# davidebarbieri/spgpu

Hardware: AMD Instinct MI355X
Metric: HELL fp64 SpMV GFLOP/s + achieved HBM GB/s (% of roofline), 1 GPU (higher is better)
Workload: dtype f64; 1 GPU; HELL fp64 SpMV (spgpuDhellspmv), 10000000 rows x 32 nnz/row uniform, hackSize 32, columns banded, alpha=1 beta=0 (BASELINE configs[1]); rows=10000000, nnz=320000000, hack_size=32, pattern=banded, parallelism=single GPU

## Files before the change

spgpu_amd/capi.py:

```python
import ctypes as C
import os

_HERE = os.path.dirname(os.path.abspath(__file__))
LIB_PATH = os.environ.get("SPGPU_LIB") or os.path.join(_HERE, "lib", "libspgpu.so")


class MissingNativeLibrary(ImportError):
    pass


if not os.path.exists(LIB_PATH):
    raise MissingNativeLibrary(
        f"{LIB_PATH} not found: build it with `make lib` (or __graft_entry__.build()); "
        "spgpu-amd has no Python or CPU fallback for its kernels")

try:
    import torch
except ImportError:
    pass

lib = C.CDLL(LIB_PATH)

SPGPU_SUCCESS, SPGPU_UNSUPPORTED, SPGPU_UNSPECIFIED, SPGPU_OUTOFMEMORY = 0, 1, 2, 3
TYPE_INT, TYPE_FLOAT, TYPE_DOUBLE, TYPE_COMPLEX_FLOAT, TYPE_COMPLEX_DOUBLE = range(5)


class FloatComplex(C.Structure):
    _fields_ = [("x", C.c_float), ("y", C.c_float)]


class DoubleComplex(C.Structure):
    _fields_ = [("x", C.c_double), ("y", C.c_double)]


class HandleStruct(C.Structure):
    _fields_ = [
        ("currentStream", C.c_void_p), ("defaultStream", C.c_void_p),
        ("device", C.c_int), ("warpSize", C.c_int), ("maxThreadsPerBlock", C.c_int),
        ("maxGridSizeX", C.c_int), ("maxGridSizeY", C.c_int), ("maxGridSizeZ", C.c_int),
        ("multiProcessorCount", C.c_int), ("capabilityMajor", C.c_int), ("capabilityMinor", C.c_int),
    ]


Handle = C.POINTER(HandleStruct)
ptr = C.c_void_p
i32 = C.c_int

SCALAR = {"S": C.c_float, "D": C.c_double, "C": FloatComplex, "Z": DoubleComplex}
REAL = {"S": C.c_float, "D": C.c_double, "C": C.c_float, "Z": C.c_double}
TYPE_CODE = {"S": TYPE_FLOAT, "D": TYPE_DOUBLE, "C": TYPE_COMPLEX_FLOAT, "Z": TYPE_COMPLEX_DOUBLE}


def scalar(letter, value):
    if letter in "SD":
        return SCALAR[letter](float(value))
    v = complex(value)
    return SCALAR[letter](v.real, v.imag)


def _bind(name, restype, argtypes):
    fn = getattr(lib, name)
    fn.restype = restype
    fn.argtypes = argtypes
    return fn


DECLARED = {}


def _decl(name, restype, argtypes):
    DECLARED[name] = (restype, argtypes)
    return _bind(name, restype, argtypes)


spgpuCreate = _decl("spgpuCreate", i32, [C.POINTER(Handle), i32])
spgpuDestroy = _decl("spgpuDestroy", None, [Handle])
spgpuStreamCreate = _decl("spgpuStreamCreate", None, [Handle, C.POINTER(C.c_void_p)])
spgpuStreamDestroy = _decl("spgpuStreamDestroy", None, [C.c_void_p])
spgpuSetStream = _decl("spgpuSetStream", None, [Handle, C.c_void_p])
spgpuGetStream = _decl("spgpuGetStream", C.c_void_p, [Handle])
spgpuSizeOf = _decl("spgpuSizeOf", C.c_size_t, [i32])

hellspmv, ellspmv, hdiaspmv = {}, {}, {}
axpby, maxpby, dot, mdot, nrm2, mnrm2 = {}, {}, {}, {}, {}, {}
for _L, _T in SCALAR.items():
    hellspmv[_L] = _decl(f"spgpu{_L}hellspmv", None,
                         [Handle, ptr, ptr, _T, ptr, ptr, i32, ptr, ptr, ptr, i32, i32, ptr, _T, i32])
    ellspmv[_L] = _decl(f"spgpu{_L}ellspmv", None,
                        [Handle, ptr, ptr, _T, ptr, ptr, i32, i32, ptr, ptr, i32, i32, i32, ptr, _T, i32])
    hdiaspmv[_L] = _decl(f"spgpu{_L}hdiaspmv", None,
                         [Handle, ptr, ptr, _T, ptr, ptr, i32, ptr, i32, i32, ptr, _T])
    axpby[_L] = _decl(f"spgpu{_L}axpby", None, [Handle, ptr, i32, _T, ptr, _T, ptr])
    maxpby[_L] = _decl(f"spgpu{_L}maxpby", None, [Handle, ptr, i32, _T, ptr, _T, ptr, i32, i32])
    dot[_L] = _decl(f"spgpu{_L}dot", _T, [Handle, i32, ptr, ptr])
    mdot[_L] = _decl(f"spgpu{_L}mdot", None, [Handle, ptr, i32, ptr, ptr, i32, i32])
    nrm2[_L] = _decl(f"spgpu{_L}nrm2", REAL[_L], [Handle, i32, ptr])
    mnrm2[_L] = _decl(f"spgpu{_L}mnrm2", None, [Handle, ptr, i32, ptr, i32, i32])

scal, vabs, axy, maxy, axypbz, maxypbz, gath, scat, setscal = {}, {}, {}, {}, {}, {}, {}, {}, {}
asum, amax, masum, mamax = {}, {}, {}, {}
for _L, _T in list(SCALAR.items()) + [("I", C.c_int)]:
    gath[_L] = _decl(f"spgpu{_L}gath", None, [Handle, ptr, i32, ptr, i32, ptr])
    scat[_L] = _decl(f"spgpu{_L}scat", None, [Handle, ptr, i32, ptr, ptr, i32, _T])
    setscal[_L] = _decl(f"spgpu{_L}setscal", None, [Handle, i32, i32, i32, _T, ptr])
    if _L == "I":
        continue
    scal[_L] = _decl(f"spgpu{_L}scal", None, [Handle, ptr, i32, _T, ptr])
    vabs[_L] = _decl(f"spgpu{_L}abs", None, [Handle, ptr, i32, _T, ptr])
    axy[_L] = _decl(f"spgpu{_L}axy", None, [Handle, ptr, i32, _T, ptr, ptr])
    maxy[_L] = _decl(f"spgpu{_L}maxy", None, [Handle, ptr, i32, _T, ptr, ptr, i32, i32])
    axypbz[_L] = _decl(f"spgpu{_L}axypbz", None, [Handle, ptr, i32, _T, ptr, _T, ptr, ptr])
    maxypbz[_L] = _decl(f"spgpu{_L}maxypbz", None, [Handle, ptr, i32, _T, ptr, _T, ptr, ptr, i32, i32])
    asum[_L] = _decl(f"spgpu{_L}asum", REAL[_L], [Handle, i32, ptr])
    amax[_L] = _decl(f"spgpu{_L}amax", REAL[_L], [Handle, i32, ptr])
    masum[_L] = _decl(f"spgpu{_L}masum", None, [Handle, ptr, i32, ptr, i32, i32])
    mamax[_L] = _decl(f"spgpu{_L}mamax", None, [Handle, ptr, i32, ptr, i32, i32])

hellspmm, mv_interleave, mv_deinterleave = {}, {}, {}
for _L in "SD":
    _T = SCALAR[_L]
    hellspmm[_L] = _decl(f"spgpu{_L}hellspmm", None,
                         [Handle, ptr, ptr, _T, ptr, ptr, i32, ptr, ptr, ptr, i32, i32, ptr, _T, i32, i32, i32, i32])
    mv_interleave[_L] = _decl(f"spgpu{_L}mvInterleave", None, [Handle, ptr, i32, ptr, i32, i32, i32])
    mv_deinterleave[_L] = _decl(f"spgpu{_L}mvDeinterleave", None, [Handle, ptr, i32, ptr, i32, i32, i32])

hellspmm_mv = {}
for _L in "SD":
    _T = SCALAR[_L]
    hellspmm_mv[_L] = _decl(f"spgpu{_L}hellspmmMv", None,
                            [Handle, ptr, ptr, _T, ptr, ptr, i32, ptr, ptr, ptr, i32, i32, ptr, _T, i32, i32, i32, i32])

computeEllRowLenghts = _decl("computeEllRowLenghts", None, [ptr, C.POINTER(i32), i32, i32, ptr, i32])
computeEllAllocPitch = _decl("computeEllAllocPitch", i32, [i32])
cooToEll = _decl("cooToEll", None, [ptr, ptr, i32, i32, i32, i32, i32, i32, ptr, ptr, ptr, i32, i32])
computeHellAllocSize = _decl("computeHellAllocSize", None, [C.POINTER(i32), i32, i32, ptr])
ellToHell = _decl("ellToHell", None, [ptr, ptr, ptr, i32, ptr, ptr, i32, i32, ptr, i32, i32])
getHdiaHacksCount = _decl("getHdiaHacksCount", i32, [i32, i32])
computeHdiaHackOffsetsFromCoo = _decl("computeHdiaHackOffsetsFromCoo", None,
                                      [C.POINTER(i32), ptr, i32, i32, i32, i32, ptr, ptr, i32])
cooToHdia = _decl("cooToHdia", None, [ptr, ptr, ptr, i32, i32, i32, i32, ptr, ptr, ptr, i32, i32])


diaspmv, ellcsput = {}, {}
for _L, _T in SCALAR.items():
    diaspmv[_L] = _decl(f"spgpu{_L}diaspmv", None, [Handle, ptr, ptr, _T, ptr, ptr, i32, i32, i32, i32, ptr, _T])
    ellcsput[_L] = _decl(f"spgpu{_L}ellcsput", None, [Handle, _T, ptr, ptr, i32, i32, ptr, i32, ptr, ptr, ptr, i32])
computeDiaAllocPitch = _decl("computeDiaAllocPitch", i32, [i32])
computeDiaDiagonalsCount = _decl("computeDiaDiagonalsCount", i32, [i32, i32, i32, ptr, ptr])
coo2dia = _decl("coo2dia", None, [ptr, ptr, i32, i32, i32, i32, i32, ptr, ptr, ptr, i32, i32])
computeHdiaHackOffsets = _decl("computeHdiaHackOffsets", None, [C.POINTER(i32), ptr, i32, ptr, i32, i32, i32, i32])
diaToHdia = _decl("diaToHdia", None, [ptr, ptr, ptr, i32, ptr, ptr, i32, i32, i32, i32])
ellToOell = _decl("ellToOell", None, [ptr, ptr, ptr, ptr, ptr, ptr, ptr, i32, i32, i32, i32])


spgpuCooConvertWorkBytes = _decl("spgpuCooConvertWorkBytes", C.c_size_t, [i32, i32])
spgpuCooRowLengthsDevice = _decl("spgpuCooRowLengthsDevice", i32, [Handle, ptr, C.POINTER(i32), i32, i32, ptr, i32, ptr])
spgpuCooToEllDevice = _decl("spgpuCooToEllDevice", i32, [Handle, ptr, ptr, i32, i32, i32, i32, i32, ptr, ptr, ptr, i32, i32, ptr, ptr])
spgpuHellPlanDevice = _decl("spgpuHellPlanDevice", i32, [Handle, C.POINTER(i32), ptr, i32, i32, ptr, ptr])
spgpuCooToHellDevice = _decl("spgpuCooToHellDevice", i32, [Handle, ptr, ptr, ptr, i32, i32, i32, i32, ptr, ptr, ptr, i32, i32, ptr, ptr])
spgpuCooDiaWorkBytes = _decl("spgpuCooDiaWorkBytes", C.c_size_t, [i32, i32])
spgpuCooDiaPlanDevice = _decl("spgpuCooDiaPlanDevice", i32, [Handle, C.POINTER(i32), i32, i32, i32, ptr, ptr, i32, ptr])
spgpuCooToDiaScratchBytes = _decl("spgpuCooToDiaScratchBytes", C.c_size_t, [i32, i32])
spgpuCooToDiaDevice = _decl("spgpuCooToDiaDevice", i32, [Handle, ptr, ptr, i32, i32, i32, i32, i32, ptr, ptr, ptr, i32, i32, ptr, ptr])
spgpuCooHdiaPlanWorkBytes = _decl("spgpuCooHdiaPlanWorkBytes", C.c_size_t, [i32, i32])
spgpuCooHdiaPlanDevice = _decl("spgpuCooHdiaPlanDevice", i32, [Handle, C.POINTER(i32), ptr, i32, i32, i32, i32, ptr, ptr, i32, ptr])
spgpuCooToHdiaScratchBytes = _decl("spgpuCooToHdiaScratchBytes", C.c_size_t, [i32, i32])
spgpuCooToHdiaDevice = _decl("spgpuCooToHdiaDevice", i32, [Handle, ptr, ptr, ptr, i32, i32, i32, i32, ptr, ptr, ptr, i32, i32, i32, ptr, ptr])


spgpuCsrRowLengthsDevice = _decl("spgpuCsrRowLengthsDevice", i32, [Handle, ptr, C.POINTER(i32), i32, ptr, i32])
spgpuCsrToEllDevice = _decl("spgpuCsrToEllDevice", i32, [Handle, ptr, ptr, i32, i32, i32, i32, ptr, ptr, ptr, i32, i32, ptr])
spgpuCsrToHellDevice = _decl("spgpuCsrToHellDevice", i32, [Handle, ptr, ptr, ptr, i32, i32, i32, ptr, ptr, ptr, i32, i32, ptr])
CSR_FILL_PLAIN, CSR_FILL_TRANSPOSE = 0, 1
spgpuCsrToEllDeviceWith = _bind("spgpuCsrToEllDeviceWith", i32, spgpuCsrToEllDevice.argtypes + [i32, i32])
spgpuCsrToHellDeviceWith = _bind("spgpuCsrToHellDeviceWith", i32, spgpuCsrToHellDevice.argtypes + [i32, i32])
CSR_FILL_CHUNK = _bind("spgpuCsrFillChunk", i32, [])()
CSR_FILL_DEFAULT = _bind("spgpuCsrDefaultFill", i32, [])()


oellOrder = _decl("oellOrder", None, [ptr, ptr, ptr, i32, i32, i32])
oellOrderAligned = _decl("oellOrderAligned", None, [ptr, ptr, ptr, i32, i32, i32])
spgpuOellOrderWorkBytes = _decl("spgpuOellOrderWorkBytes", C.c_size_t, [i32])
spgpuOellOrderDevice = _decl("spgpuOellOrderDevice", i32, [Handle, ptr, ptr, ptr, i32, i32, i32, ptr])
spgpuOellOrderAlignedDevice = _decl("spgpuOellOrderAlignedDevice", i32, [Handle, ptr, ptr, ptr, i32, i32, i32, ptr])
spgpuEllToOellDevice = _decl("spgpuEllToOellDevice", i32, [Handle, ptr, ptr, ptr, ptr, ptr, ptr, ptr, i32, i32, i32, i32, i32, i32, ptr])
spgpuCooPermuteRowsDevice = _decl("spgpuCooPermuteRowsDevice", i32, [Handle, ptr, ptr, i32, ptr, i32, i32, ptr])


class HellBlockD(C.Structure):
    _fields_ = [("cM", C.c_void_p), ("rP", C.c_void_p), ("hackSize", C.c_int), ("hackOffsets", C.c_void_p), ("rS", C.c_void_p),
                ("rows", C.c_int), ("avgNnzPerRow", C.c_int), ("baseIndex", C.c_int), ("slots", C.c_longlong)]


EXCHANGE_ALLGATHER, EXCHANGE_NEEDED = 0, 1
ShardedPlan = C.c_void_p
spgpuCommAvailable = _decl("spgpuCommAvailable", i32, [])
spgpuCommGetUniqueId = _decl("spgpuCommGetUniqueId", i32, [ptr])
spgpuCommInitRank = _decl("spgpuCommInitRank", i32, [C.POINTER(C.c_void_p), i32, ptr, i32])
spgpuCommInitAll = _decl("spgpuCommInitAll", i32, [C.POINTER(C.c_void_p), i32, ptr])
spgpuCommDestroy = _decl("spgpuCommDestroy", None, [ptr])
spgpuDhellspmmShardedCreate = _decl("spgpuDhellspmmShardedCreate", i32,
                                    [C.POINTER(ShardedPlan), Handle, ptr, i32, i32, C.POINTER(C.c_longlong), C.POINTER(HellBlockD),
                                     C.POINTER(HellBlockD), i32, i32])
spgpuDhellspmmShardedStep = _decl("spgpuDhellspmmShardedStep", i32, [ShardedPlan, ptr, ptr, C.c_double, ptr, C.c_double])
spgpuDhellspmmShardedExchange = _decl("spgpuDhellspmmShardedExchange", i32, [ShardedPlan, ptr])
spgpuDhellspmmShardedExchangeWait = _decl("spgpuDhellspmmShardedExchangeWait", i32, [ShardedPlan])
spgpuDhellspmmShardedProducts = _decl("spgpuDhellspmmShardedProducts", i32, [ShardedPlan, ptr, ptr, C.c_double, ptr, C.c_double])
spgpuDhellspmmShardedRowsReceived = _decl("spgpuDhellspmmShardedRowsReceived", C.c_longlong, [ShardedPlan])
spgpuDhellspmmShardedExchanged = _decl("spgpuDhellspmmShardedExchanged", C.c_void_p, [ShardedPlan, C.POINTER(C.c_longlong)])
spgpuDhellspmmShardedDestroy = _decl("spgpuDhellspmmShardedDestroy", None, [ShardedPlan])


def hell_block(part, avg_nnz=0):
    p = lambda t: t.data_ptr()
    slots = int(part["slots"]) if "slots" in part else int(part["cM"].numel())
    return HellBlockD(p(part["cM"]), p(part["rP"]), part["hack_size"], p(part["hack_offsets"]), p(part["rS"]), part["rows"], avg_nnz,
                      part.get("base", 0), slots)


spgpuMmProperties = _decl("spgpuMmProperties", i32, [C.c_char_p, ptr])
spgpuMmReadCoo = _decl("spgpuMmReadCoo", i32, [C.c_char_p, C.c_char, ptr, ptr, ptr])
spgpuMmUnfoldedSizeD = _decl("spgpuMmUnfoldedSizeD", i32, [ptr, ptr, ptr, i32])
spgpuMmUnfoldD = _decl("spgpuMmUnfoldD", None, [ptr, ptr, ptr, ptr, ptr, ptr, i32])


dot_device, axpby_device, axpby_quot_device, div_device, nrm2_device = {}, {}, {}, {}, {}
for _L in "SD":
    dot_device[_L] = _decl(f"spgpu{_L}dotDevice", None, [Handle, ptr, i32, ptr, ptr])
    nrm2_device[_L] = _decl(f"spgpu{_L}nrm2Device", None, [Handle, ptr, i32, ptr])
    axpby_device[_L] = _decl(f"spgpu{_L}axpbyDevice", None, [Handle, ptr, i32, ptr, ptr, ptr, ptr])
    axpby_quot_device[_L] = _decl(f"spgpu{_L}axpbyQuotDevice", None, [Handle, ptr, i32, ptr, ptr, ptr, ptr, ptr, i32, ptr])
    div_device[_L] = _decl(f"spgpu{_L}divDevice", None, [Handle, ptr, ptr, ptr, i32])
hellspmv_dot_device, axpby_pair_dot_device = {}, {}
for _L in "SD":
    _S = SCALAR[_L]
    hellspmv_dot_device[_L] = _decl(f"spgpu{_L}hellspmvDotDevice", None,
                                    [Handle, ptr, ptr, ptr, ptr, _S, ptr, ptr, i32, ptr, ptr, i32, ptr, _S, i32])
    axpby_pair_dot_device[_L] = _decl(f"spgpu{_L}axpbyPairDotDevice", None,
                                      [Handle, ptr, i32, ptr, ptr, ptr, ptr, ptr, ptr, ptr, ptr])


FORM_AUTO, FORM_GATHER, FORM_STRIPS, FORM_XTILE, FORM_SWEEP = range(5)
spgpuSetSpmvForm = _decl("spgpuSetSpmvForm", None, [Handle, i32])
spgpuGetSpmvForm = _decl("spgpuGetSpmvForm", i32, [Handle])
spgpuDeepListOverflows = _decl("spgpuDeepListOverflows", i32, [Handle])
spgpuDeepListFallbacks = _decl("spgpuDeepListFallbacks", i32, [Handle])
spgpuDeepListsRecycled = _decl("spgpuDeepListsRecycled", i32, [Handle])
spgpuSpmvPlanCounts = _decl("spgpuSpmvPlanCounts", None, [Handle, C.POINTER(i32), C.POINTER(i32), C.POINTER(i32)])
spgpuHellSpmvPrepare = _decl("spgpuHellSpmvPrepare", i32, [Handle, i32, ptr, ptr, i32, ptr, ptr, ptr, i32, i32])
spgpuHellSpmvFreeze = _decl("spgpuHellSpmvFreeze", i32, [Handle, i32, ptr, ptr, i32, ptr, ptr, ptr, i32, i32])
spgpuEllSpmvFreeze = _decl("spgpuEllSpmvFreeze", i32, [Handle, i32, ptr, ptr, i32, i32, ptr, ptr, i32, i32, i32])
spgpuHellSpmvAdopt = _decl("spgpuHellSpmvAdopt", i32, [Handle, i32, ptr, ptr, i32, ptr, ptr, i32, i32])
spgpuEllSpmvAdopt = _decl("spgpuEllSpmvAdopt", i32, [Handle, i32, ptr, ptr, i32, i32, ptr, i32, i32, i32])
spgpuHellSpmvOptimize = _decl("spgpuHellSpmvOptimize", i32, [Handle, i32, ptr, ptr, i32, ptr, ptr, ptr, i32, i32])
SPMV_AS_IS, SPMV_FROZEN, SPMV_ADOPTED = 0, 1, 2
spgpuSpmvAdoptedUses = _decl("spgpuSpmvAdoptedUses", i32, [Handle])
spgpuSpmvThaw = _decl("spgpuSpmvThaw", i32, [Handle, ptr])
spgpuSpmvFrozenBytes = _decl("spgpuSpmvFrozenBytes", C.c_longlong, [Handle])
spgpuEllSpmvPrepare = _decl("spgpuEllSpmvPrepare", i32, [Handle, i32, ptr, ptr, i32, i32, ptr, ptr, i32, i32, i32])

SPGPU_IN_USE = 4
spgpuSpmvHold = _decl("spgpuSpmvHold", i32, [Handle, ptr])
spgpuSpmvRelease = _decl("spgpuSpmvRelease", i32, [Handle, ptr])
spgpuSpmvHolds = _decl("spgpuSpmvHolds", i32, [Handle, ptr])


def plan_counts(handle):
    u, b, s = i32(0), i32(0), i32(0)
    spgpuSpmvPlanCounts(handle, C.byref(u), C.byref(b), C.byref(s))
    return u.value, b.value, s.value
spgpuGetLastSpmvForm = _decl("spgpuGetLastSpmvForm", i32, [Handle])
spgpuTuningVariantsBuilt = _decl("spgpuTuningVariantsBuilt", i32, [])
spgpuHellSpmvForm = _decl("spgpuHellSpmvForm", i32, [Handle, i32, ptr, i32, ptr, ptr, i32, i32])
spgpuEllSpmvForm = _decl("spgpuEllSpmvForm", i32, [Handle, i32, ptr, i32, ptr, i32, i32, i32])

spgpuTuningReload = _decl("spgpuTuningReload", None, [])


def create_handle(device=0):
    h = Handle()
    status = spgpuCreate(C.byref(h), device)
    if status != SPGPU_SUCCESS or not h:
        raise RuntimeError(f"spgpuCreate(device={device}) failed with status {status}")
    return h
```

spgpu_amd/csrc/core.c:

```c
#include "spgpu_internal.h"

#include <stdio.h>
#include <stdlib.h>
#include <string.h>

#define DEEP_HEAD_BYTES (SPGPU_DEEP_HEAD_INTS * sizeof(int))
#define DEEP_ENTRY_BYTES ((size_t)SPGPU_DEEP_ENTRIES * sizeof(SpgpuDeepEntry))
#define DEEP_ITEM_ENTRY_BYTES ((size_t)SPGPU_DEEP_ITEMS * sizeof(SpgpuDeepItem))
#define DEEP_PARTIAL_BYTES ((size_t)SPGPU_DEEP_ENTRIES * 32 * 16)
#define DEEP_ITEM_SUM_BYTES ((size_t)SPGPU_DEEP_ITEMS * 32 * 16)

static void deepListFor(SpgpuPrivateHandle* h, hipStream_t stream)
{
    pthread_mutex_lock(&h->tablesLock);
    int known = 0;
    for (int i = 0; i < h->deepStreams; ++i)
        known |= h->deepStream[i] == stream;
    if (!known && h->deepStreams < SPGPU_DEEP_STREAMS) {
        void* p = NULL;
        hipEvent_t idle = NULL;
        if (hipMalloc(&p, DEEP_HEAD_BYTES + DEEP_ENTRY_BYTES + DEEP_ITEM_ENTRY_BYTES + DEEP_PARTIAL_BYTES + DEEP_ITEM_SUM_BYTES) == hipSuccess) {
            if (spgpuTuning()->poisonScratch)
                (void)hipMemset((char*)p + DEEP_HEAD_BYTES + DEEP_ENTRY_BYTES + DEEP_ITEM_ENTRY_BYTES, 0xFF, DEEP_PARTIAL_BYTES + DEEP_ITEM_SUM_BYTES);
            if (hipMemset(p, 0, DEEP_HEAD_BYTES + DEEP_ENTRY_BYTES + DEEP_ITEM_ENTRY_BYTES) == hipSuccess &&
                hipEventCreateWithFlags(&idle, hipEventDisableTiming) == hipSuccess) {
                h->deepScratch[h->deepStreams] = p;
                h->deepStream[h->deepStreams] = stream;
                h->deepIdle[h->deepStreams] = idle;
                h->deepUsed[h->deepStreams] = 0;
                h->deepPinned[h->deepStreams] = 0;
                h->deepClock[h->deepStreams] = ++h->deepTick;
                h->deepStreams += 1;
            } else {
                hipFree(p);
            }
        }
    } else if (!known) {
        int pick = -1;
        for (int i = 0; i < h->deepStreams; ++i) {
            if (h->deepStream[i] == h->pub.defaultStream || h->deepPinned[i])
                continue;
            if (h->deepUsed[i] && !spgpuEventDone(h->deepIdle[i]))
                continue;
            if (pick < 0 || h->deepClock[i] < h->deepClock[pick])
                pick = i;
        }
        if (pick >= 0) {
            h->deepStream[pick] = stream;
            h->deepUsed[pick] = 0;
            h->deepClock[pick] = ++h->deepTick;
            h->deepRecycled += 1;
        }
    }
    pthread_mutex_unlock(&h->tablesLock);
}

spgpuStatus_t spgpuCreate(spgpuHandle_t* pHandle, int device)
{
    if (!pHandle)
        return SPGPU_UNSPECIFIED;
    *pHandle = NULL;

    hipDeviceProp_t prop;
    hipError_t perr = hipGetDeviceProperties(&prop, device);
    if (perr != hipSuccess) {
        fprintf(stderr, "spgpuCreate: hipGetDeviceProperties(%d) failed: %s\n", device, hipGetErrorString(perr));
        return SPGPU_UNSPECIFIED;
    }

    SpgpuPrivateHandle* h = (SpgpuPrivateHandle*)calloc(1, sizeof(SpgpuPrivateHandle));
    if (!h)
        return SPGPU_OUTOFMEMORY;

    int previous = 0;
    hipGetDevice(&previous);
    hipError_t err = hipSetDevice(device);
    if (err == hipSuccess)
        err = hipStreamCreate(&h->pub.defaultStream);
    if (err == hipSuccess)
        err = hipMalloc(&h->reduceScratch, SPGPU_REDUCE_SCRATCH_BYTES);
    if (err == hipSuccess && spgpuTuning()->poisonScratch)
        err = hipMemset(h->reduceScratch, 0xFF, SPGPU_REDUCE_SCRATCH_BYTES);
    if (err == hipSuccess)
        err = hipHostMalloc(&h->reduceHost, SPGPU_REDUCE_SCRATCH_BYTES, hipHostMallocDefault);
    if (err == hipSuccess)
        err = hipHostMalloc((void**)&h->formFeedback, (SPGPU_FEEDBACK_ENTRIES + 2) * SPGPU_FEEDBACK_SAMPLES * sizeof(int),
                            hipHostMallocDefault);
    if (err == hipSuccess)
        memset(h->formFeedback, 0, (SPGPU_FEEDBACK_ENTRIES + 2) * SPGPU_FEEDBACK_SAMPLES * sizeof(int));
    hipSetDevice(previous);

    if (err != hipSuccess) {
        fprintf(stderr, "spgpuCreate: device %d setup failed: %s\n", device, hipGetErrorString(err));
        if (h->reduceScratch) hipFree(h->reduceScratch);
        if (h->reduceHost) hipHostFree(h->reduceHost);
        if (h->pub.defaultStream) hipStreamDestroy(h->pub.defaultStream);
        free(h);
        return err == hipErrorOutOfMemory ? SPGPU_OUTOFMEMORY : SPGPU_UNSPECIFIED;
    }

    h->pub.currentStream = h->pub.defaultStream;
    h->pub.device = device;
    h->pub.warpSize = prop.warpSize;
    h->pub.maxThreadsPerBlock = prop.maxThreadsPerBlock;
    h->pub.maxGridSizeX = prop.maxGridSize[0];
    h->pub.maxGridSizeY = prop.maxGridSize[1];
    h->pub.maxGridSizeZ = prop.maxGridSize[2];
    h->pub.multiProcessorCount = prop.multiProcessorCount;
    h->pub.capabilityMajor = prop.major;
    h->pub.capabilityMinor = prop.minor;
    h->magic = SPGPU_HANDLE_MAGIC;
    pthread_mutex_init(&h->tablesLock, NULL);
    h->spmvForm = SPGPU_SPMV_FORM_AUTO;
    hipSetDevice(device);
    deepListFor(h, h->pub.defaultStream);
    spgpuRecordsCreate(h);
    hipSetDevice(previous);

    *pHandle = &h->pub;
    return SPGPU_SUCCESS;
}

void spgpuDestroy(spgpuHandle_t pHandle)
{
    if (!pHandle)
        return;
    SpgpuPrivateHandle* h = spgpuPrivate(pHandle);
    int previous = 0;
    hipGetDevice(&previous);
    hipSetDevice(h->pub.device);
    hipDeviceSynchronize();
    hipFree(h->reduceScratch);
    for (int i = 0; i < h->deepStreams; ++i) {
        hipFree(h->deepScratch[i]);
        hipEventDestroy(h->deepIdle[i]);
    }
    spgpuRecordsDestroy(h);
    hipHostFree(h->reduceHost);
    hipHostFree(h->formFeedback);
    hipStreamDestroy(h->pub.defaultStream);
    hipSetDevice(previous);
    pthread_mutex_destroy(&h->tablesLock);
    h->magic = 0;
    free(h);
}

void spgpuStreamCreate(spgpuHandle_t pHandle, hipStream_t* stream)
{
    int previous = 0;
    hipGetDevice(&previous);
    hipSetDevice(pHandle->device);
    hipStreamCreate(stream);
    hipSetDevice(previous);
}

void spgpuStreamDestroy(hipStream_t stream)
{
    hipStreamDestroy(stream);
}

void spgpuSetStream(spgpuHandle_t pHandle, hipStream_t stream)
{
    SpgpuPrivateHandle* h = spgpuPrivate(pHandle);
    h->pub.currentStream = stream ? stream : h->pub.defaultStream;
    int known = 0;
    pthread_mutex_lock(&h->tablesLock);
    for (int i = 0; i < h->deepStreams; ++i)
        known |= h->deepStream[i] == h->pub.currentStream;
    pthread_mutex_unlock(&h->tablesLock);
    if (!known) {
        int previous = 0;
        hipGetDevice(&previous);
        hipSetDevice(h->pub.device);
        deepListFor(h, h->pub.currentStream);
        hipSetDevice(previous);
    }
}

hipStream_t spgpuGetStream(spgpuHandle_t pHandle)
{
    return pHandle->currentStream;
}

size_t spgpuSizeOf(spgpuType_t typeCode)
{
    switch (typeCode) {
    case SPGPU_TYPE_INT:            return sizeof(int);
    case SPGPU_TYPE_FLOAT:          return sizeof(float);
    case SPGPU_TYPE_DOUBLE:         return sizeof(double);
    case SPGPU_TYPE_COMPLEX_FLOAT:  return sizeof(hipFloatComplex);
    case SPGPU_TYPE_COMPLEX_DOUBLE: return sizeof(hipDoubleComplex);
    default:                        return 0;
    }
}

spgpuStatus_t spgpuDeepScratch(spgpuHandle_t pHandle, SpgpuDeepList* list)
{
    SpgpuPrivateHandle* h = spgpuPrivate(pHandle);
    char* base = NULL;
    pthread_mutex_lock(&h->tablesLock);
    for (int i = 0; i < h->deepStreams; ++i)
        if (h->deepStream[i] == h->pub.currentStream) {
            base = (char*)h->deepScratch[i];
            list->idle = h->deepIdle[i];
            h->deepUsed[i] = 1;
            h->deepClock[i] = ++h->deepTick;
        }
    if (!base)
        h->deepFallbacks += 1;
    pthread_mutex_unlock(&h->tablesLock);
    if (!base)
        return SPGPU_UNSUPPORTED;
    list->header = (int*)base;
    list->entries = (SpgpuDeepEntry*)(base + DEEP_HEAD_BYTES);
    list->items = (SpgpuDeepItem*)(base + DEEP_HEAD_BYTES + DEEP_ENTRY_BYTES);
    list->partials = base + DEEP_HEAD_BYTES + DEEP_ENTRY_BYTES + DEEP_ITEM_ENTRY_BYTES;
    list->itemSums = base + DEEP_HEAD_BYTES + DEEP_ENTRY_BYTES + DEEP_ITEM_ENTRY_BYTES + DEEP_PARTIAL_BYTES;
    return SPGPU_SUCCESS;
}

void spgpuDeepListPin(spgpuHandle_t pHandle)
{
    SpgpuPrivateHandle* h = spgpuPrivate(pHandle);
    pthread_mutex_lock(&h->tablesLock);
    for (int i = 0; i < h->deepStreams; ++i)
        if (h->deepStream[i] == h->pub.currentStream)
            h->deepPinned[i] = 1;
    pthread_mutex_unlock(&h->tablesLock);
}

int* spgpuAnalyseWords(spgpuHandle_t pHandle)
{
    return spgpuPrivate(pHandle)->formFeedback + SPGPU_FEEDBACK_ENTRIES * SPGPU_FEEDBACK_SAMPLES;
}

int* spgpuDeepOverflowWords(spgpuHandle_t pHandle)
{
    return spgpuPrivate(pHandle)->formFeedback + (SPGPU_FEEDBACK_ENTRIES + 1) * SPGPU_FEEDBACK_SAMPLES;
}

int spgpuDeepListOverflows(spgpuHandle_t pHandle)
{
    return ((volatile int*)spgpuDeepOverflowWords(pHandle))[0];
}

int spgpuDeepListFallbacks(spgpuHandle_t pHandle)
{
    SpgpuPrivateHandle* h = spgpuPrivate(pHandle);
    pthread_mutex_lock(&h->tablesLock);
    const int n = h->deepFallbacks;
    pthread_mutex_unlock(&h->tablesLock);
    return n;
}

int spgpuDeepListsRecycled(spgpuHandle_t pHandle)
{
    SpgpuPrivateHandle* h = spgpuPrivate(pHandle);
    pthread_mutex_lock(&h->tablesLock);
    const int n = h->deepRecycled;
    pthread_mutex_unlock(&h->tablesLock);
    return n;
}

void spgpuSetSpmvForm(spgpuHandle_t pHandle, int form)
{
    if (form < SPGPU_SPMV_FORM_AUTO || form > SPGPU_SPMV_FORM_SWEEP)
        form = SPGPU_SPMV_FORM_AUTO;
    __atomic_store_n(&spgpuPrivate(pHandle)->spmvForm, form, __ATOMIC_RELAXED);
}

int spgpuGetSpmvForm(spgpuHandle_t pHandle)
{
    return __atomic_load_n(&spgpuPrivate(pHandle)->spmvForm, __ATOMIC_RELAXED);
}

int spgpuGetLastSpmvForm(spgpuHandle_t pHandle)
{
    return __atomic_load_n(&spgpuPrivate(pHandle)->lastSpmvForm, __ATOMIC_RELAXED);
}

void spgpuNoteSpmvForm(spgpuHandle_t pHandle, int form)
{
    __atomic_store_n(&spgpuPrivate(pHandle)->lastSpmvForm, form, __ATOMIC_RELAXED);
}

static SpgpuTuning tuning;
static int tuningLoaded;

static int envInt(const char* name, int fallback)
{
    const char* s = getenv(name);
    return s && *s ? atoi(s) : fallback;
}

void spgpuTuningReload(void)
{
    SpgpuTuning t;
    t.xStrips = envInt("SPGPU_X_STRIPS", -1);
    t.autoSweep = envInt("SPGPU_AUTO_SWEEP", 1);
    t.poisonScratch = envInt("SPGPU_POISON_SCRATCH", 0);
    t.deepSplit = envInt("SPGPU_DEEP_SPLIT", -1);
    t.deepCap = envInt("SPGPU_DEEP_CAP", 256);
    t.deepKeep = envInt("SPGPU_DEEP_KEEP", 64);
    t.raggedShape = envInt("SPGPU_RAGGED_SHAPE", 0);
    t.raggedSplit = envInt("SPGPU_RAGGED_SPLIT", -1);
    t.plan = envInt("SPGPU_PLAN", 1);
    t.freezeEscapesPct = envInt("SPGPU_FREEZE_MAX_ESCAPES_PCT", 1);
    tuning = t;
    __atomic_store_n(&tuningLoaded, 1, __ATOMIC_RELEASE);
}

const SpgpuTuning* spgpuTuning(void)
{
    if (!__atomic_load_n(&tuningLoaded, __ATOMIC_ACQUIRE))
        spgpuTuningReload();
    return &tuning;
}
```

spgpu_amd/csrc/ellpack_spmv.hip:

```cpp
#include "numeric.hip.h"
#include <type_traits>
#include "spgpu_internal.h"
#include "slab_args.hip.h"

#include "spgpu/ell.h"
#include "spgpu/hell.h"

#include <stdio.h>
#include <stdlib.h>

namespace spgpu {

#include "slab_spmv.hip.h"
#include "deep_items.hip.h"
#include "form_probe.hip.h"
#include "sweep_spmv.hip.h"

#ifdef SPGPU_TRACE_BLOCKS
__device__ unsigned long long* spgpuTraceBuffer;
#endif
#include "ragged_spmv.hip.h"


static bool alignedTo(const void* p, size_t bytes)
{
    return ((uintptr_t)p % bytes) == 0;
}

template <typename T, int RPL, int PH, bool IS_HELL, bool NT, int UNROLL, bool PIPE, bool TAIL, bool STRIPS = false,
          int BLOCK = kBlockThreads, int TILE_BYTES = 0, int TAIL_EVERY = 0, bool PACKED = false>
static void launchSlabKernel(hipStream_t stream, const SlabArgs<T>& a)
{
    constexpr int GROUP_ROWS = (kWave / PH) * RPL;
    constexpr int WAVES = BLOCK / kWave;
    const long long groups = ((long long)a.rows + GROUP_ROWS - 1) / GROUP_ROWS;
    const unsigned blocks = (unsigned)((groups + WAVES - 1) / WAVES);
    hipLaunchKernelGGL((slabSpmvKernel<T, RPL, PH, IS_HELL, NT, UNROLL, PIPE, TAIL, STRIPS, BLOCK, TILE_BYTES, TAIL_EVERY, PACKED>),
                       dim3(blocks), dim3(BLOCK), 0, stream, a);
}

template <typename T, int RPL, bool IS_HELL>
static void launchTiled(hipStream_t stream, const SlabArgs<T>& a)
{
    constexpr int PH = sizeof(T) == 16 ? 2 : 1;
    if constexpr (sizeof(T) == 4 && RPL == 4)
        launchSlabKernel<T, RPL, 2 * RPL, IS_HELL, true, 2, true, true, false, 512, 32768>(stream, a);
    else if constexpr (sizeof(T) == 8 && RPL == 2)
        launchSlabKernel<T, RPL, 1, IS_HELL, true, 4, true, true, false, 256, 32768, 8>(stream, a);
    else
        launchSlabKernel<T, RPL, PH, IS_HELL, true, 4, true, PH == 1, false, 256, 32768>(stream, a);
}

constexpr int kAutoSweepRows = 2 * 1024 * 1024;

template <typename T, int VEC, bool IS_HELL>
static void launchSweep(hipStream_t stream, const SlabArgs<T>& a)
{
    constexpr int PACKS = sizeof(T) == 16 ? 16 : 32 / VEC;
    constexpr bool TAIL = sizeof(T) == 8;
    const long long packs = ((long long)a.rows + VEC - 1) / VEC;
    long long blocks = (packs + (long long)kBlockThreads * PACKS - 1) / ((long long)kBlockThreads * PACKS);
    blocks = blocks > 2048 ? 2048 : blocks;
    if (isNotZero(a.beta))
        hipLaunchKernelGGL((sweepSpmvKernel<T, VEC, PACKS, IS_HELL, true, TAIL>), dim3((unsigned)blocks), dim3(kBlockThreads), 0, stream, a);
    else
        hipLaunchKernelGGL((sweepSpmvKernel<T, VEC, PACKS, IS_HELL, false, TAIL>), dim3((unsigned)blocks), dim3(kBlockThreads), 0, stream, a);
}

template <typename T, int RPL, bool IS_HELL>
static void launchDeep(hipStream_t stream, const SlabArgs<T>& a)
{
    constexpr int PH = kWave / (32 / RPL);
    constexpr int UNROLL = 32 / PH;
    hipLaunchKernelGGL((deepItemsKernel<T, RPL, IS_HELL, UNROLL, kDeepChunk>), dim3(SPGPU_DEEP_ITEMS / (kBlockThreads / kWave)), dim3(kBlockThreads), 0, stream, a);
    hipLaunchKernelGGL((deepFinishKernel<T>), dim3(256), dim3(kBlockThreads), 0, stream, a);
}

template <typename T, int RPL, bool IS_HELL>
static void launchLean(hipStream_t stream, const SlabArgs<T>& a)
{
    launchSlabKernel<T, RPL, 1, IS_HELL, true, 4, false, true, false, kBlockThreads, 0, 8>(stream, a);
}

template <typename T, bool IS_HELL>
static void launchFormProbe(hipStream_t stream, const SlabArgs<T>& a, bool wideOk)
{
    constexpr int WIDE = 16 / (int)sizeof(T);
    if constexpr (WIDE > 1) {
        if (wideOk) {
            if constexpr (sizeof(T) == 4)
                hipLaunchKernelGGL((formProbeKernel<T, WIDE, 2 * WIDE, IS_HELL, 2 * WIDE * 2>), dim3(3), dim3(kWave), 0, stream, a);
            else
                hipLaunchKernelGGL((formProbeKernel<T, WIDE, 1, IS_HELL, 8>), dim3(3), dim3(kWave), 0, stream, a);
            return;
        }
    }
    hipLaunchKernelGGL((formProbeKernel<T, 1, 2, IS_HELL, 8>), dim3(3), dim3(kWave), 0, stream, a);
}

#include "frozen_slab.hip.h"

template <typename T> constexpr int kWide = 16 / (int)sizeof(T);
template <typename T> constexpr int kWideGroupRows = sizeof(T) == 4 ? (kWave / (2 * kWide<T>)) * kWide<T> : kWave * kWide<T>;

template <typename T, bool IS_HELL>
static bool wideLayout(const SlabArgs<T>& a)
{
    constexpr int WIDE = 16 / (int)sizeof(T);
    const long long stripRows = ((long long)a.rows + WIDE - 1) / WIDE * WIDE;
    const bool layoutOk = IS_HELL ? (a.hackSize > 0 && a.hackSize % WIDE == 0)
                                  : (a.valStride >= stripRows && a.idxStride >= stripRows);
    return layoutOk && alignedTo(a.cM, 16) && alignedTo(a.rP, 4 * WIDE) && a.valStride % WIDE == 0 && a.idxStride % WIDE == 0;
}

template <typename T>
static bool attachDeepList(spgpuHandle_t handle, SlabArgs<T>& a, bool wideOk, SpgpuDeepList* list, bool* noDeepList)
{
    const SpgpuTuning* tune = spgpuTuning();
    const bool deepSplit = (tune->deepSplit >= 0 ? tune->deepSplit != 0 : a.rIdx != nullptr) && wideOk;
    a.deepCap = tune->deepCap > 0 ? tune->deepCap : 256;
    a.deepKeep = tune->deepKeep >= 0 && tune->deepKeep < a.deepCap ? tune->deepKeep : a.deepCap;
    a.deepChunk = kDeepChunk;
    a.deepOverflow = spgpuDeepOverflowWords(handle);
    *noDeepList = false;
    list->idle = nullptr;
    if (!deepSplit)
        return false;
    if (spgpuDeepScratch(handle, list) == SPGPU_SUCCESS) {
        a.deepHeader = list->header;
        a.deepEntries = list->entries;
        a.deepItems = list->items;
        a.deepPartials = static_cast<T*>(list->partials);
        a.deepItemSums = static_cast<T*>(list->itemSums);
    } else {
        *noDeepList = true;
    }
    return true;
}

template <typename T, bool IS_HELL>
static int orderedShape(spgpuHandle_t handle, hipStream_t stream, const SlabArgs<T>& a, bool wait)
{
    int calls = 0, tag = 0;
    int* seen = spgpuFormFeedback(handle, a.rP, a.rows, &calls, &tag);
    int said = spgpuFeedbackSaid(((volatile int*)seen)[3], tag);
    if (said == 0 || calls % 64 == 0)
        hipLaunchKernelGGL((orderedProbeKernel<IS_HELL>), dim3(1), dim3(kWave), 0, stream, a.rP, a.rS, a.hackOffsets, a.rIdx, a.hackSize,
                           a.idxStride, a.maxNnz, a.rows, a.baseIndex, seen + 3, tag);
    if (wait && said == 0 && hipStreamSynchronize(stream) == hipSuccess)
        said = spgpuFeedbackSaid(((volatile int*)seen)[3], tag);
    return said == 4 || said == 6 ? 4 : 0;
}

template <typename T, bool IS_HELL>
static bool launchOrdered(spgpuHandle_t handle, hipStream_t stream, SlabArgs<T>& a, int form, const SpgpuDeepList& list, bool noDeepList, SpmvCall call)
{
    constexpr int WIDE = 16 / (int)sizeof(T);
    const bool tiledForm = form != SPGPU_SPMV_FORM_GATHER;
    spgpuNoteSpmvForm(handle, tiledForm ? SPGPU_SPMV_FORM_XTILE : SPGPU_SPMV_FORM_GATHER);
    int shape = spgpuTuning()->raggedShape;
    if (shape == 0 && tiledForm && a.rIdx != nullptr && sizeof(T) <= 8)
        shape = orderedShape<T, IS_HELL>(handle, stream, a, call != SpmvCall::Run);
    if (noDeepList && shape != 4)
        shape = 0;
    const bool plannable = !tiledForm || shape == 0 || shape == 4;
    if (call != SpmvCall::Run)
        return plannable && launchPlanned<T, IS_HELL>(handle, stream, a, shape, tiledForm, false, call);
    if (plannable && launchPlanned<T, IS_HELL>(handle, stream, a, shape, tiledForm, noDeepList, SpmvCall::Run))
        return true;
    const bool deepPossible = IS_HELL || a.maxNnz > a.deepCap;
    const bool deepKernels = launchRagged<T, WIDE, IS_HELL, true>(stream, a, shape, tiledForm);
    if (deepPossible && deepKernels)
        launchDeep<T, WIDE, IS_HELL>(stream, a);
    if (list.idle) {
        if (!spgpuStreamCapturing(stream))
            (void)hipEventRecord(list.idle, stream);
        else
            spgpuDeepListPin(handle);
    }
    return true;
}

struct FormVote {
    bool strips, autoTile, autoSweep, probeBehind;
};

template <typename T>
static FormVote voteForm(spgpuHandle_t handle, SlabArgs<T>& a, int form, bool eligible)
{
    FormVote vote{false, false, false, false};
    a.feedback = nullptr;
    a.tileSpanLimit = (long long)(32768 / sizeof(T)) * 5 / 4;
    if (!eligible)
        return vote;
    if (form != SPGPU_SPMV_FORM_AUTO) {
        vote.strips = form == SPGPU_SPMV_FORM_STRIPS;
        return vote;
    }
    int calls = 0, tag = 0;
    int* seen = spgpuFormFeedback(handle, a.rP, a.rows, &calls, &tag);
    a.feedbackTag = tag;
    int gathers = 0, local = 0, sweeps = 0;
    for (int q = 0; q < 3; ++q) {
        const int said = spgpuFeedbackSaid(((volatile int*)seen)[q], tag);
        gathers += said == 1 ? 1 : 0;
        local += said == 3 ? 1 : 0;
        sweeps += said == 4 ? 1 : 0;
    }
    vote.autoTile = local >= 2;
    vote.strips = gathers + local + sweeps < 2;
    vote.autoSweep = sweeps >= 2 && !vote.autoTile && sizeof(T) == 8 && spgpuTuning()->autoSweep != 0 && !a.rIdx && a.rows >= kAutoSweepRows;
    a.feedback = seen;
    vote.probeBehind = !vote.strips && (calls % 4 == 0 || calls == 1);
    return vote;
}

template <typename T, bool IS_HELL>
static void launchRowsAsTheyCome(spgpuHandle_t handle, hipStream_t stream, SlabArgs<T>& a, int form, bool wideOk, bool tiled, const FormVote& vote)
{
    constexpr int WIDE = 16 / (int)sizeof(T);
    constexpr bool PHASED = sizeof(T) == 4;
    spgpuNoteSpmvForm(handle, (tiled || vote.autoTile) ? SPGPU_SPMV_FORM_XTILE
                                                       : (vote.autoSweep ? SPGPU_SPMV_FORM_SWEEP : (vote.strips ? SPGPU_SPMV_FORM_STRIPS : SPGPU_SPMV_FORM_GATHER)));
    if (vote.probeBehind)
        launchFormProbe<T, IS_HELL>(stream, a, wideOk);
    if (vote.autoSweep) {
        if constexpr (WIDE > 1) {
            a.wideIO = alignedTo(a.z, 16) && alignedTo(a.y, 16);
            a.feedback = nullptr;
            launchSweep<T, WIDE, IS_HELL>(stream, a);
            return;
        }
    }
    if (!vote.strips)
        a.feedback = nullptr;
    if (wideOk) {
        a.wideIO = alignedTo(a.z, 16) && alignedTo(a.y, 16);
        if constexpr (WIDE > 1) {
            if (tiled || vote.autoTile) {
                launchTiled<T, WIDE, IS_HELL>(stream, a);
            } else if (!PHASED && a.avgNnzPerRow > 0 && a.avgNnzPerRow <= 8 && form == SPGPU_SPMV_FORM_AUTO && (IS_HELL || a.maxNnz <= 16)) {
                spgpuNoteSpmvForm(handle, SPGPU_SPMV_FORM_GATHER);
                a.feedback = nullptr;
                launchLean<T, WIDE, IS_HELL>(stream, a);
            } else {
                findFrozenSlab(handle, stream, a, kWideGroupRows<T>);
                constexpr int PH = PHASED ? 2 * WIDE : 1, UNROLL = PHASED ? 2 : 8;
                if (a.planPacked && vote.strips)
                    launchSlabKernel<T, WIDE, PH, IS_HELL, true, UNROLL, true, true, true, kBlockThreads, 0, 0, true>(stream, a);
                else if (a.planPacked)
                    launchSlabKernel<T, WIDE, PH, IS_HELL, true, UNROLL, true, true, false, kBlockThreads, 0, 0, true>(stream, a);
                else if (vote.strips)
                    launchSlabKernel<T, WIDE, PH, IS_HELL, true, UNROLL, true, true, true>(stream, a);
                else
                    launchSlabKernel<T, WIDE, PH, IS_HELL, true, UNROLL, true, true>(stream, a);
            }
            return;
        }
    }
    a.wideIO = 1;
    if (tiled)
        launchTiled<T, 1, IS_HELL>(stream, a);
    else
        launchSlabKernel<T, 1, 2, IS_HELL, true, 4, true, false>(stream, a);
}

template <typename T, bool IS_HELL>
static bool launchSlabFamily(spgpuHandle_t handle, const SlabArgs<T>& in, SpmvCall call = SpmvCall::Run)
{
    if (in.rows <= 0)
        return false;
    SlabArgs<T> a = in;
    hipStream_t stream = handle->currentStream;
    constexpr int WIDE = 16 / (int)sizeof(T);
    const bool wideOk = wideLayout<T, IS_HELL>(a);
    a.tailLanes = kTailLanes;
    int form = spgpuGetSpmvForm(handle);
    if (spgpuTuning()->xStrips >= 0)
        form = spgpuTuning()->xStrips ? SPGPU_SPMV_FORM_STRIPS : SPGPU_SPMV_FORM_GATHER;
    if (form == SPGPU_SPMV_FORM_SWEEP) {
        if (wideOk && !a.rIdx) {
            if (call != SpmvCall::Run)
                return false;
            a.wideIO = alignedTo(a.z, 16) && alignedTo(a.y, 16);
            a.feedback = nullptr;
            spgpuNoteSpmvForm(handle, SPGPU_SPMV_FORM_SWEEP);
            launchSweep<T, WIDE, IS_HELL>(stream, a);
            return true;
        }
        form = SPGPU_SPMV_FORM_AUTO;
    }
    const bool tiled = form == SPGPU_SPMV_FORM_XTILE;
    SpgpuDeepList list;
    bool noDeepList;
    if (attachDeepList(handle, a, wideOk, &list, &noDeepList))
        return launchOrdered<T, IS_HELL>(handle, stream, a, form, list, noDeepList, call);
    if (call != SpmvCall::Run) {
        if constexpr (WIDE > 1) {
            if (call == SpmvCall::Freeze && !a.rIdx && wideOk && !tiled)
                return freezeSlab<IS_HELL>(handle, stream, planKey(a, nullptr, 0, -kWideGroupRows<T>));
        }
        return false;
    }
    const FormVote vote = voteForm(handle, a, form, wideOk && WIDE > 1 && !tiled);
    launchRowsAsTheyCome<T, IS_HELL>(handle, stream, a, form, wideOk, tiled, vote);
    return true;
}

template <typename T>
static SlabArgs<T> matrixArgs(const void* cM, const int* rP, int hackSize, const int* hackOffsets, long long valStride, long long idxStride,
                              const int* rS, const int* rIdx, int maxNnz, int rows, int baseIndex)
{
    SlabArgs<T> a{};
    a.cM = static_cast<const T*>(cM);
    a.rP = rP;
    a.rS = rS;
    a.rIdx = rIdx;
    a.hackOffsets = hackOffsets;
    a.rows = rows;
    a.baseIndex = baseIndex;
    a.hackSize = hackSize;
    a.maxNnz = maxNnz;
    a.valStride = valStride;
    a.idxStride = idxStride;
    return a;
}

template <typename T, bool IS_HELL, typename ApiT>
static void runSpmv(spgpuHandle_t handle, SlabArgs<T>& a, ApiT* z, const ApiT* y, ApiT alpha, const ApiT* x, ApiT beta, int avgNnzPerRow)
{
    static_assert(sizeof(T) == sizeof(ApiT), "ABI type and device type must have one layout");
    a.z = reinterpret_cast<T*>(z);
    a.y = reinterpret_cast<const T*>(y);
    a.x = reinterpret_cast<const T*>(x);
    __builtin_memcpy(&a.alpha, &alpha, sizeof(T));
    __builtin_memcpy(&a.beta, &beta, sizeof(T));
    a.avgNnzPerRow = avgNnzPerRow;
    (void)launchSlabFamily<T, IS_HELL>(handle, a);
}

template <typename T, typename ApiT>
static void hellSpmv(spgpuHandle_t handle, ApiT* z, const ApiT* y, ApiT alpha, const ApiT* cM, const int* rP,
                     int hackSize, const int* hackOffsets, const int* rS, const int* rIdx, int rows,
                     const ApiT* x, ApiT beta, int baseIndex, int avgNnzPerRow = 0)
{
    if (!rIdx) {
        const SpgpuAdopted* copy = spgpuAdoptedFind(handle, handle->currentStream, cM, rP, rS, hackOffsets, rows, hackSize, baseIndex, 0, 0);
        if (copy && spgpuSizeOf((spgpuType_t)copy->type) == sizeof(T)) {
            cM = static_cast<const ApiT*>(copy->values);
            rP = copy->indices;
            hackOffsets = copy->hackOffsetsOrdered;
            rS = copy->lengths;
            rIdx = copy->order;
        }
    }
    SlabArgs<T> a = matrixArgs<T>(cM, rP, hackSize, hackOffsets, hackSize, hackSize, rS, rIdx, 0, rows, baseIndex);
    runSpmv<T, true>(handle, a, z, y, alpha, x, beta, avgNnzPerRow);
    spgpuDebugCheck(handle, "hellspmv");
}

template <typename T, typename ApiT>
static void ellSpmv(spgpuHandle_t handle, ApiT* z, const ApiT* y, ApiT alpha, const ApiT* cM, const int* rP,
                    int cMPitch, int rPPitch, const int* rS, const int* rIdx, int maxNnzPerRow, int rows,
                    const ApiT* x, ApiT beta, int baseIndex, int avgNnzPerRow = 0)
{
    if (!rIdx && rS) {
        const SpgpuAdopted* copy = spgpuAdoptedFind(handle, handle->currentStream, cM, rP, rS, nullptr, rows, 0, baseIndex, cMPitch, rPPitch);
        if (copy && spgpuSizeOf((spgpuType_t)copy->type) == sizeof(T)) {
            hellSpmv<T, ApiT>(handle, z, y, alpha, static_cast<const ApiT*>(copy->values), copy->indices, 32, copy->hackOffsetsOrdered, copy->lengths,
                              copy->order, rows, x, beta, baseIndex, avgNnzPerRow);
            return;
        }
    }
    SlabArgs<T> a = matrixArgs<T>(cM, rP, 0, nullptr, cMPitch, rPPitch, rS, rIdx, maxNnzPerRow, rows, baseIndex);
    runSpmv<T, false>(handle, a, z, y, alpha, x, beta, avgNnzPerRow);
    spgpuDebugCheck(handle, "ellspmv");
}

template <typename T, bool IS_HELL>
static int prepareSpmv(spgpuHandle_t handle, const void* cM, const int* rP, int hackSize, const int* hackOffsets, long long valStride, long long idxStride,
                       const int* rS, const int* rIdx, int maxNnz, int rows, int baseIndex, bool freeze)
{
    const SlabArgs<T> a = matrixArgs<T>(cM, rP, hackSize, hackOffsets, valStride, idxStride, rS, rIdx, maxNnz, rows, baseIndex);
    return launchSlabFamily<T, IS_HELL>(handle, a, freeze ? SpmvCall::Freeze : SpmvCall::Prepare) ? SPGPU_SUCCESS : SPGPU_UNSUPPORTED;
}

template <bool IS_HELL>
static int prepareSpmvOfType(spgpuHandle_t handle, spgpuType_t type, const void* cM, const int* rP, int hackSize, const int* hackOffsets, long long valStride,
                             long long idxStride, const int* rS, const int* rIdx, int maxNnz, int rows, int baseIndex, bool freeze = false)
{
    if (!handle || !rP || !cM || rows < 0)
        return SPGPU_UNSPECIFIED;
    switch (type) {
    case SPGPU_TYPE_FLOAT: return prepareSpmv<float, IS_HELL>(handle, cM, rP, hackSize, hackOffsets, valStride, idxStride, rS, rIdx, maxNnz, rows, baseIndex, freeze);
    case SPGPU_TYPE_DOUBLE: return prepareSpmv<double, IS_HELL>(handle, cM, rP, hackSize, hackOffsets, valStride, idxStride, rS, rIdx, maxNnz, rows, baseIndex, freeze);
    case SPGPU_TYPE_COMPLEX_FLOAT: return prepareSpmv<cfloat, IS_HELL>(handle, cM, rP, hackSize, hackOffsets, valStride, idxStride, rS, rIdx, maxNnz, rows, baseIndex, freeze);
    case SPGPU_TYPE_COMPLEX_DOUBLE: return prepareSpmv<cdouble, IS_HELL>(handle, cM, rP, hackSize, hackOffsets, valStride, idxStride, rS, rIdx, maxNnz, rows, baseIndex, freeze);
    default: return SPGPU_UNSPECIFIED;
    }
}

#include "ell_csput.hip.h"

template <typename T, typename ApiT>
static void ellCsput(spgpuHandle_t handle, ApiT* cM, const int* rP, int cMPitch, int rPPitch, const int* rS, int nnz,
                     const int* aI, const int* aJ, const ApiT* aVal, int baseIndex)
{
    if (nnz <= 0)
        return;
    const unsigned blocks = (unsigned)(((long long)nnz + kBlockThreads - 1) / kBlockThreads);
    hipLaunchKernelGGL((ellCsputKernel<T>), dim3(blocks), dim3(kBlockThreads), 0, handle->currentStream,
                       reinterpret_cast<T*>(cM), rP, (long long)cMPitch, (long long)rPPitch, rS, nnz, aI, aJ,
                       reinterpret_cast<const T*>(aVal), baseIndex);
    spgpuDebugCheck(handle, "ellcsput");
}

template <typename T, bool IS_HELL>
static int analyseForm(spgpuHandle_t handle, const int* rP, int hackSize, const int* hackOffsets, long long idxStride, const int* rS,
                       int maxNnz, int rows, int baseIndex)
{
    if (rows <= 0)
        return SPGPU_SPMV_FORM_GATHER;
    constexpr int WIDE = 16 / (int)sizeof(T);
    SlabArgs<T> a = matrixArgs<T>(nullptr, rP, hackSize, hackOffsets, idxStride, idxStride, rS, nullptr, maxNnz, rows, baseIndex);
    a.tileSpanLimit = (long long)(32768 / sizeof(T)) * 5 / 4;
    int* seen = spgpuAnalyseWords(handle);
    seen[0] = seen[1] = seen[2] = 0;
    a.feedback = seen;
    a.feedbackTag = 0;
    const bool wide = IS_HELL ? (hackSize > 0 && hackSize % WIDE == 0) : true;
    launchFormProbe<T, IS_HELL>(handle->currentStream, a, wide);
    if (hipStreamSynchronize(handle->currentStream) != hipSuccess)
        return SPGPU_SPMV_FORM_AUTO;
    int strips = 0, local = 0, sweeps = 0;
    for (int q = 0; q < 3; ++q) {
        strips += seen[q] == 2;
        local += seen[q] == 3;
        sweeps += seen[q] == 4;
    }
    if (sweeps >= 2 && sizeof(T) == 8 && rows >= kAutoSweepRows)
        return SPGPU_SPMV_FORM_SWEEP;
    return strips >= 2 ? SPGPU_SPMV_FORM_STRIPS : (local >= 2 ? SPGPU_SPMV_FORM_XTILE : SPGPU_SPMV_FORM_GATHER);
}

template <bool IS_HELL>
static int analyseFormOfType(spgpuHandle_t handle, spgpuType_t type, const int* rP, int hackSize, const int* hackOffsets, long long idxStride,
                             const int* rS, int maxNnz, int rows, int baseIndex)
{
    switch (type) {
    case SPGPU_TYPE_FLOAT: return analyseForm<float, IS_HELL>(handle, rP, hackSize, hackOffsets, idxStride, rS, maxNnz, rows, baseIndex);
    case SPGPU_TYPE_DOUBLE: return analyseForm<double, IS_HELL>(handle, rP, hackSize, hackOffsets, idxStride, rS, maxNnz, rows, baseIndex);
    case SPGPU_TYPE_COMPLEX_FLOAT: return analyseForm<cfloat, IS_HELL>(handle, rP, hackSize, hackOffsets, idxStride, rS, maxNnz, rows, baseIndex);
    case SPGPU_TYPE_COMPLEX_DOUBLE: return analyseForm<cdouble, IS_HELL>(handle, rP, hackSize, hackOffsets, idxStride, rS, maxNnz, rows, baseIndex);
    default: return SPGPU_SPMV_FORM_AUTO;
    }
}

}

using namespace spgpu;

extern "C" {

int spgpuTuningVariantsBuilt(void)
{
    return 0;
}

int spgpuHellSpmvForm(spgpuHandle_t handle, spgpuType_t type, const int* rP, int hackSize, const int* hackOffsets, const int* rS, int rows,
                      int baseIndex)
{
    return analyseFormOfType<true>(handle, type, rP, hackSize, hackOffsets, hackSize, rS, 0, rows, baseIndex);
}

int spgpuHellSpmvPrepare(spgpuHandle_t handle, spgpuType_t type, const void* cM, const int* rP, int hackSize, const int* hackOffsets, const int* rS,
                         const int* rIdx, int rows, int baseIndex)
{
    if (!hackOffsets || !rS || hackSize <= 0)
        return SPGPU_UNSPECIFIED;
    return spgpu::prepareSpmvOfType<true>(handle, type, cM, rP, hackSize, hackOffsets, hackSize, hackSize, rS, rIdx, 0, rows, baseIndex);
}

int spgpuEllSpmvPrepare(spgpuHandle_t handle, spgpuType_t type, const void* cM, const int* rP, int cMPitch, int rPPitch, const int* rS, const int* rIdx,
                        int maxNnzPerRow, int rows, int baseIndex)
{
    return spgpu::prepareSpmvOfType<false>(handle, type, cM, rP, 0, nullptr, cMPitch, rPPitch, rS, rIdx, maxNnzPerRow, rows, baseIndex);
}

int spgpuHellSpmvFreeze(spgpuHandle_t handle, spgpuType_t type, const void* cM, const int* rP, int hackSize, const int* hackOffsets, const int* rS,
                        const int* rIdx, int rows, int baseIndex)
{
    if (!hackOffsets || !rS || hackSize <= 0)
        return SPGPU_UNSPECIFIED;
    return spgpu::prepareSpmvOfType<true>(handle, type, cM, rP, hackSize, hackOffsets, hackSize, hackSize, rS, rIdx, 0, rows, baseIndex, true);
}

int spgpuEllSpmvFreeze(spgpuHandle_t handle, spgpuType_t type, const void* cM, const int* rP, int cMPitch, int rPPitch, const int* rS, const int* rIdx,
                       int maxNnzPerRow, int rows, int baseIndex)
{
    return spgpu::prepareSpmvOfType<false>(handle, type, cM, rP, 0, nullptr, cMPitch, rPPitch, rS, rIdx, maxNnzPerRow, rows, baseIndex, true);
}

int spgpuEllSpmvForm(spgpuHandle_t handle, spgpuType_t type, const int* rP, int rPPitch, const int* rS, int maxNnzPerRow, int rows,
                     int baseIndex)
{
    return analyseFormOfType<false>(handle, type, rP, 0, nullptr, rPPitch, rS, maxNnzPerRow, rows, baseIndex);
}

#ifdef SPGPU_TRACE_BLOCKS
void spgpuPlannedSetTrace(unsigned long long* buffer);
void spgpuDebugSetTrace(unsigned long long* buffer)
{
    (void)hipMemcpyToSymbol(HIP_SYMBOL(spgpu::spgpuTraceBuffer), &buffer, sizeof(buffer));
    spgpuPlannedSetTrace(buffer);
}
#endif

void spgpuDebugCheck(spgpuHandle_t h, const char* what)
{
#ifdef SPGPU_DEBUG
    hipError_t err = hipStreamSynchronize(h->currentStream);
    if (err == hipSuccess)
        err = hipGetLastError();
    if (err != hipSuccess) {
        fprintf(stderr, "spgpu: HIP error in %s: %s\n", what, hipGetErrorString(err));
        exit(1);
    }
#else
    (void)h;
    (void)what;
#endif
}


void spgpuShellspmv(spgpuHandle_t handle, float* z, const float* y, float alpha, const float* cM,
                    const int* rP, int hackSize, const int* hackOffsets, const int* rS, const int* rIdx,
                    int avgNnzPerRow, int rows, const float* x, float beta, int baseIndex)
{
    hellSpmv<float>(handle, z, y, alpha, cM, rP, hackSize, hackOffsets, rS, rIdx, rows, x, beta, baseIndex, avgNnzPerRow);
}

void spgpuDhellspmv(spgpuHandle_t handle, double* z, const double* y, double alpha, const double* cM,
                    const int* rP, int hackSize, const int* hackOffsets, const int* rS, const int* rIdx,
                    int avgNnzPerRow, int rows, const double* x, double beta, int baseIndex)
{
    hellSpmv<double>(handle, z, y, alpha, cM, rP, hackSize, hackOffsets, rS, rIdx, rows, x, beta, baseIndex, avgNnzPerRow);
}

void spgpuChellspmv(spgpuHandle_t handle, hipFloatComplex* z, const hipFloatComplex* y, hipFloatComplex alpha,
                    const hipFloatComplex* cM, const int* rP, int hackSize, const int* hackOffsets,
                    const int* rS, const int* rIdx, int avgNnzPerRow, int rows, const hipFloatComplex* x,
                    hipFloatComplex beta, int baseIndex)
{
    hellSpmv<cfloat>(handle, z, y, alpha, cM, rP, hackSize, hackOffsets, rS, rIdx, rows, x, beta, baseIndex, avgNnzPerRow);
}

void spgpuZhellspmv(spgpuHandle_t handle, hipDoubleComplex* z, const hipDoubleComplex* y,
                    hipDoubleComplex alpha, const hipDoubleComplex* cM, const int* rP, int hackSize,
                    const int* hackOffsets, const int* rS, const int* rIdx, int avgNnzPerRow, int rows,
                    const hipDoubleComplex* x, hipDoubleComplex beta, int baseIndex)
{
    hellSpmv<cdouble>(handle, z, y, alpha, cM, rP, hackSize, hackOffsets, rS, rIdx, rows, x, beta, baseIndex, avgNnzPerRow);
}

void spgpuSellspmv(spgpuHandle_t handle, float* z, const float* y, float alpha, const float* cM, const int* rP,
                   int cMPitch, int rPPitch, const int* rS, const int* rIdx, int avgNnzPerRow,
                   int maxNnzPerRow, int rows, const float* x, float beta, int baseIndex)
{
    ellSpmv<float>(handle, z, y, alpha, cM, rP, cMPitch, rPPitch, rS, rIdx, maxNnzPerRow, rows, x, beta, baseIndex, avgNnzPerRow);
}

void spgpuDellspmv(spgpuHandle_t handle, double* z, const double* y, double alpha, const double* cM,
                   const int* rP, int cMPitch, int rPPitch, const int* rS, const int* rIdx, int avgNnzPerRow,
                   int maxNnzPerRow, int rows, const double* x, double beta, int baseIndex)
{
    ellSpmv<double>(handle, z, y, alpha, cM, rP, cMPitch, rPPitch, rS, rIdx, maxNnzPerRow, rows, x, beta, baseIndex, avgNnzPerRow);
}

void spgpuCellspmv(spgpuHandle_t handle, hipFloatComplex* z, const hipFloatComplex* y, hipFloatComplex alpha,
                   const hipFloatComplex* cM, const int* rP, int cMPitch, int rPPitch, const int* rS,
                   const int* rIdx, int avgNnzPerRow, int maxNnzPerRow, int rows, const hipFloatComplex* x,
                   hipFloatComplex beta, int baseIndex)
{
    ellSpmv<cfloat>(handle, z, y, alpha, cM, rP, cMPitch, rPPitch, rS, rIdx, maxNnzPerRow, rows, x, beta, baseIndex, avgNnzPerRow);
}

void spgpuZellspmv(spgpuHandle_t handle, hipDoubleComplex* z, const hipDoubleComplex* y, hipDoubleComplex alpha,
                   const hipDoubleComplex* cM, const int* rP, int cMPitch, int rPPitch, const int* rS,
                   const int* rIdx, int avgNnzPerRow, int maxNnzPerRow, int rows, const hipDoubleComplex* x,
                   hipDoubleComplex beta, int baseIndex)
{
    ellSpmv<cdouble>(handle, z, y, alpha, cM, rP, cMPitch, rPPitch, rS, rIdx, maxNnzPerRow, rows, x, beta, baseIndex, avgNnzPerRow);
}

void spgpuSellcsput(spgpuHandle_t handle, float alpha, float* cM, const int* rP, int cMPitch, int rPPitch, const int* rS,
                    int nnz, int* aI, int* aJ, float* aVal, int baseIndex)
{
    (void)alpha;
    ellCsput<float>(handle, cM, rP, cMPitch, rPPitch, rS, nnz, aI, aJ, aVal, baseIndex);
}
void spgpuDellcsput(spgpuHandle_t handle, double alpha, double* cM, const int* rP, int cMPitch, int rPPitch,
                    const int* rS, int nnz, int* aI, int* aJ, double* aVal, int baseIndex)
{
    (void)alpha;
    ellCsput<double>(handle, cM, rP, cMPitch, rPPitch, rS, nnz, aI, aJ, aVal, baseIndex);
}
void spgpuCellcsput(spgpuHandle_t handle, hipFloatComplex alpha, hipFloatComplex* cM, const int* rP, int cMPitch,
                    int rPPitch, const int* rS, int nnz, int* aI, int* aJ, hipFloatComplex* aVal, int baseIndex)
{
    (void)alpha;
    ellCsput<cfloat>(handle, cM, rP, cMPitch, rPPitch, rS, nnz, aI, aJ, aVal, baseIndex);
}
void spgpuZellcsput(spgpuHandle_t handle, hipDoubleComplex alpha, hipDoubleComplex* cM, const int* rP, int cMPitch,
                    int rPPitch, const int* rS, int nnz, int* aI, int* aJ, hipDoubleComplex* aVal, int baseIndex)
{
    (void)alpha;
    ellCsput<cdouble>(handle, cM, rP, cMPitch, rPPitch, rS, nnz, aI, aJ, aVal, baseIndex);
}

}
```

spgpu_amd/csrc/slab_spmv.hip.h:

```cpp

template <typename E, int N> __device__ inline E* ldsArray()
{
    __shared__ __attribute__((aligned(16))) E buffer[N];
    return buffer;
}

__device__ inline long long sampleGroup(long long groups, int q)
{
    const long long at = groups * q / 4 + 2 * q + 1;
    return at < groups ? at : groups - 1;
}

template <typename T, int RPL, int PH, bool IS_HELL, bool NT, int UNROLL, bool PIPE, bool TAIL, bool STRIPS = false,
          int BLOCK = kBlockThreads, int TILE_BYTES = 0, int TAIL_EVERY = 0, bool PACKED = false>
__global__ __launch_bounds__(BLOCK) void slabSpmvKernel(const SlabArgs<T> a)
{
    static_assert(!PACKED || (TILE_BYTES == 0 && RPL >= 2), "packed indices: the gather and strip forms of 4- and 8-byte elements");
    using ColumnWord = typename std::conditional<PACKED, unsigned short, int>::type;
    constexpr int LPC = kWave / PH;
    constexpr int GROUP_ROWS = LPC * RPL;
    constexpr int WAVES = BLOCK / kWave;
    constexpr bool XTILE = TILE_BYTES > 0;
    constexpr int TILE_ELEMS = TILE_BYTES / (int)sizeof(T);

    const int lane = threadIdx.x & (kWave - 1);
    const int sub = lane % LPC;
    const int phase = lane / LPC;
    const T* __restrict__ x = a.x;
    auto groupOf = [&]() -> long long {
        const int wave = threadIdx.x >> 6;
        return (long long)blockIdx.x * WAVES + wave;
    };

    T* tile = nullptr;
    int tileBase = 0;
    unsigned tileCount = 0;
    if constexpr (XTILE) {
        tile = ldsArray<T, TILE_ELEMS>();
        ColumnProbe mine{0x7fffffff, -0x7fffffff - 1, 0, 0};
        if (phase == 0) {
            int first[RPL], last[RPL], lenAt[RPL];
#pragma unroll
            for (int once = 0; once < 1; ++once) {
                const long long r0 = groupOf() * GROUP_ROWS + (long long)sub * RPL;
                long long at = 0;
                if (r0 < a.rows) {
                    if constexpr (IS_HELL) {
                        const unsigned u0 = (unsigned)r0, hs = (unsigned)a.hackSize;
                        at = (long long)a.hackOffsets[u0 / hs] + (u0 % hs);
                    } else {
                        at = r0;
                    }
                }
#pragma unroll
                for (int t = 0; t < RPL; ++t) {
                    const long long r = r0 + t;
                    lenAt[t] = r < a.rows ? (a.rS ? a.rS[r] : a.maxNnz) : 0;
                    first[t] = lenAt[t] > 0 ? a.rP[at + t] : 0;
                    last[t] = lenAt[t] > 0 ? a.rP[at + t + (long long)(lenAt[t] - 1) * a.idxStride] : 0;
                }
            }
#pragma unroll
            for (int t = 0; t < RPL; ++t) {
                if (lenAt[t] > 0) {
                    const int f = first[t] - a.baseIndex, l = last[t] - a.baseIndex;
                    const int low = f < l ? f : l, high = f < l ? l : f;
                    mine.lowest = low < mine.lowest ? low : mine.lowest;
                    mine.highest = high > mine.highest ? high : mine.highest;
                    mine.middles += ((long long)f + l) >> 1;
                    mine.rows += 1;
                }
            }
        }
        mine.lowest = waveMin(mine.lowest);
        mine.highest = waveMax(mine.highest);
#pragma unroll
        for (int m = 1; m < kWave; m <<= 1) {
            mine.rows += laneXor(mine.rows, m);
            const int lowHalf = laneXor((int)(unsigned)(mine.middles & 0xffffffffll), m);
            const int highHalf = laneXor((int)(mine.middles >> 32), m);
            mine.middles += ((long long)highHalf << 32) | (unsigned)lowHalf;
        }
        ColumnProbe* seen = ldsArray<ColumnProbe, WAVES>();
        if (lane == 0)
            seen[threadIdx.x >> 6] = mine;
        __syncthreads();
        ColumnProbe all{0x7fffffff, -0x7fffffff - 1, 0, 0};
#pragma unroll
        for (int w = 0; w < WAVES; ++w) {
            const ColumnProbe other = seen[w];
            all.lowest = other.lowest < all.lowest ? other.lowest : all.lowest;
            all.highest = other.highest > all.highest ? other.highest : all.highest;
            all.rows += other.rows;
            all.middles += other.middles;
        }
        if (all.rows > 0 && all.lowest >= 0) {
            const long long span = (long long)all.highest - all.lowest + 1;
            if (span <= TILE_ELEMS) {
                tileBase = all.lowest;
                tileCount = (unsigned)span;
            } else {
                long long start = all.middles / all.rows - TILE_ELEMS / 2;
                start = start < all.lowest ? all.lowest : start;
                start = start + TILE_ELEMS > (long long)all.highest + 1 ? (long long)all.highest + 1 - TILE_ELEMS : start;
                tileBase = (int)start;
                tileCount = TILE_ELEMS;
            }
        }
        constexpr int PIECE = 16 / (int)sizeof(T);
        const T* __restrict__ from = x + tileBase;
        const unsigned pieces = tileCount / PIECE;
        for (unsigned p0 = threadIdx.x; p0 < pieces; p0 += 4u * BLOCK) {
            Pack<T, PIECE> w[4];
#pragma unroll
            for (int q = 0; q < 4; ++q)
                if (p0 + q * BLOCK < pieces)
                    w[q] = loadPackElementAligned<T, PIECE>(from + (size_t)(p0 + q * BLOCK) * PIECE);
#pragma unroll
            for (int q = 0; q < 4; ++q)
                if (p0 + q * BLOCK < pieces)
                    storePack<T, PIECE>(tile + (size_t)(p0 + q * BLOCK) * PIECE, w[q]);
        }
        if (pieces * PIECE + threadIdx.x < tileCount)
            tile[pieces * PIECE + threadIdx.x] = from[pieces * PIECE + threadIdx.x];
        __syncthreads();
    }

    auto processGroup = [&](const long long group) {
    const long long groupRow0 = group * GROUP_ROWS;
    if (groupRow0 >= a.rows)
        return;
    const long long row0 = groupRow0 + (long long)sub * RPL;
    const bool stripLive = row0 < a.rows;

    long long slab = 0;
    if (stripLive) {
        if constexpr (IS_HELL) {
            const unsigned r0 = (unsigned)row0, hs = (unsigned)a.hackSize;
            const unsigned hack = r0 / hs;
            slab = (long long)a.hackOffsets[hack] + (r0 - hack * hs);
        } else {
            slab = row0;
        }
    }

    int len[RPL];
    int laneLongest = 0;
#pragma unroll
    for (int t = 0; t < RPL; ++t) {
        const long long r = row0 + t;
        len[t] = r < a.rows ? (a.rS ? a.rS[r] : a.maxNnz) : 0;
        laneLongest = len[t] > laneLongest ? len[t] : laneLongest;
    }
    const int groupLongest = waveMax(laneLongest);

    T sum[RPL];
#pragma unroll
    for (int t = 0; t < RPL; ++t)
        sum[t] = zeroOf<T>();

    const T* __restrict__ vals = a.cM + slab;
    const int* __restrict__ idxs = a.rP + slab;
    int packBase = 0;
    if constexpr (PACKED)
        packBase = a.packBases[group];

    struct Stage {
        Pack<T, RPL> v[UNROLL];
        Pack<ColumnWord, RPL> c[UNROLL];
    };
    auto fetch = [&](int kBase, Stage& s) {
#pragma unroll
        for (int u = 0; u < UNROLL; ++u) {
            const int k = kBase + u * PH + phase;
            if (k < laneLongest) {
                s.v[u] = loadPack<NT, T, RPL>(vals + (long long)k * a.valStride);
                if constexpr (PACKED)
                    s.c[u] = loadPack<NT, unsigned short, RPL>(a.planPacked + slab + (long long)k * a.idxStride);
                else
                    s.c[u] = loadPack<NT, int, RPL>(idxs + (long long)k * a.idxStride);
            } else {
#pragma unroll
                for (int t = 0; t < RPL; ++t) {
                    s.v[u].v[t] = zeroOf<T>();
                    s.c[u].v[t] = PACKED ? (ColumnWord)0xFFFF : (ColumnWord)a.baseIndex;
                }
            }
        }
    };
    auto columnOf = [&](const Stage& s, int u, int t, int k) -> int {
        if constexpr (PACKED) {
            const unsigned word = s.c[u].v[t];
            if (word == 0xFFFFu)
                return k < len[t] ? idxs[t + (long long)k * a.idxStride] - a.baseIndex : 0;
            return packBase + (int)word;
        } else {
            return s.c[u].v[t] - a.baseIndex;
        }
    };
    auto consume = [&](auto stripsTag, int kBase, const Stage& s, auto&& between) {
        constexpr bool AS_STRIPS = decltype(stripsTag)::value;
        T xv[UNROLL][RPL];
        bool use[UNROLL][RPL];
#pragma unroll
        for (int u = 0; u < UNROLL; ++u) {
            const int k = kBase + u * PH + phase;
            if constexpr (AS_STRIPS) {
                const bool present = k < len[0];
                const Pack<T, RPL> w = loadPackElementAligned<T, RPL>(present ? x + (PACKED ? packBase + (int)s.c[u].v[0] : (int)s.c[u].v[0] - a.baseIndex) : a.cM);
#pragma unroll
                for (int t = 0; t < RPL; ++t) {
                    use[u][t] = present;
                    xv[u][t] = w.v[t];
                }
            } else if constexpr (XTILE) {
                bool outside = false;
                unsigned at[RPL];
#pragma unroll
                for (int t = 0; t < RPL; ++t) {
                    const int col = s.c[u].v[t] - a.baseIndex;
                    use[u][t] = k < len[t] && col >= 0;
                    at[t] = (unsigned)(col - tileBase);
                    const bool inside = at[t] < tileCount;
                    outside |= use[u][t] && !inside;
                    xv[u][t] = tile[inside ? at[t] : 0u];
                }
                if (__ballot(outside) != 0ull) {
#pragma unroll
                    for (int t = 0; t < RPL; ++t) {
                        if (use[u][t] && at[t] >= tileCount)
                            xv[u][t] = x[s.c[u].v[t] - a.baseIndex];
                    }
                }
            } else {
#pragma unroll
                for (int t = 0; t < RPL; ++t) {
                    const int col = columnOf(s, u, t, k);
                    use[u][t] = k < len[t] && col >= 0;
                    xv[u][t] = x[use[u][t] ? col : 0];
                }
            }
        }
        between();
#pragma unroll
        for (int u = 0; u < UNROLL; ++u) {
#pragma unroll
            for (int t = 0; t < RPL; ++t) {
                sum[t] = pick(use[u][t], mulAdd(s.v[u].v[t], xv[u][t], sum[t]), sum[t]);
            }
        }
    };
    auto stageIsStrips = [&](int kBase, const Stage& s) -> bool {
        bool scattered = false;
#pragma unroll
        for (int u = 0; u < UNROLL; ++u) {
            const int k = kBase + u * PH + phase;
            const bool present = k < len[0];
#pragma unroll
            for (int t = 0; t < RPL; ++t) {
                if constexpr (PACKED)
                    scattered |= (k < len[t]) != present ||
                                 (present && (s.c[u].v[t] == 0xFFFFu || (unsigned)s.c[u].v[t] != (unsigned)s.c[u].v[0] + (unsigned)t));
                else
                    scattered |= (k < len[t]) != present ||
                                 (present && (s.c[u].v[0] - a.baseIndex < 0 || s.c[u].v[t] != s.c[u].v[0] + t));
            }
        }
        return __ballot(scattered) == 0ull;
    };

    auto columnSpan = [&]() -> long long {
        int lowest = 0x7fffffff, highest = -1;
        bool below = false;
        if (phase == 0) {
#pragma unroll
            for (int t = 0; t < RPL; ++t) {
                if (len[t] > 0) {
                    const int f = idxs[t] - a.baseIndex, l = idxs[t + (long long)(len[t] - 1) * a.idxStride] - a.baseIndex;
                    below |= f < 0 || l < 0;
                    lowest = f < lowest ? f : lowest;
                    lowest = l < lowest ? l : lowest;
                    highest = f > highest ? f : highest;
                    highest = l > highest ? l : highest;
                }
            }
        }
        lowest = waveMin(lowest);
        highest = waveMax(highest);
        if (__ballot(below) != 0ull)
            return 1ll << 40;
        return highest < lowest ? 0ll : (long long)highest - lowest + 1;
    };

    constexpr int STEP = PH * UNROLL;
    int tailFrom = groupLongest;
    constexpr int TAIL_STRIDE = TAIL_EVERY > 0 ? TAIL_EVERY : PH * UNROLL;
    auto switchToTail = [&](int kBase) -> bool {
        if constexpr (TAIL) {
            if (kBase % TAIL_STRIDE == 0 && __popcll(__ballot(kBase < laneLongest)) <= a.tailLanes) {
                tailFrom = kBase;
                return true;
            }
        }
        return false;
    };
    constexpr bool STRIPS_POSSIBLE = STRIPS && RPL > 1;
    int kBase = 0;
    bool done = false;
    if constexpr (PIPE) {
        Stage cur, nxt;
        fetch(0, cur);
        auto stage = [&](auto form) {
            consume(form, kBase, cur, [&] { fetch(kBase + STEP, nxt); });
            cur = nxt;
        };
        if constexpr (STRIPS_POSSIBLE) {
            for (; kBase < groupLongest; kBase += STEP) {
                if (switchToTail(kBase)) {
                    done = true;
                    break;
                }
                if (!stageIsStrips(kBase, cur))
                    break;
                stage(std::true_type{});
            }
            if (a.feedback) {
                const long long groups = ((long long)a.rows + GROUP_ROWS - 1) / GROUP_ROWS;
                if (group == sampleGroup(groups, 1) || group == sampleGroup(groups, 2) || group == sampleGroup(groups, 3)) {
                    const int other = groupLongest > STEP && columnSpan() <= a.tileSpanLimit ? 3 : 1;
                    for (int q = 1; q <= 3; ++q)
                        if (group == sampleGroup(groups, q) && lane == 0)
                            a.feedback[q - 1] = a.feedbackTag | (2 * kBase >= groupLongest && groupLongest > STEP ? 2 : other);
                }
            }
        }
        if (!done) {
            for (kBase = __builtin_amdgcn_readfirstlane(kBase); kBase < groupLongest; kBase += STEP) {
                if (switchToTail(kBase))
                    break;
                stage(std::false_type{});
            }
        }
    } else {
        for (; kBase < groupLongest; kBase += STEP) {
            if (switchToTail(kBase))
                break;
            Stage cur;
            fetch(kBase, cur);
            consume(std::false_type{}, kBase, cur, [] {});
        }
    }

    if constexpr (TAIL) {
        unsigned long long pending = __ballot(tailFrom < laneLongest);
        while (pending) {
            const int owner = (__ffsll((long long)pending) - 1) % LPC;
            pending &= ~__ballot(sub == owner);
            const long long ownerSlab = __shfl(slab, owner, kWave);
#pragma unroll
            for (int t = 0; t < RPL; ++t) {
                const int rowLen = __shfl(len[t], owner, kWave);
                if (rowLen <= tailFrom)
                    continue;
                const T* __restrict__ rowVals = a.cM + ownerSlab + t;
                const int* __restrict__ rowIdxs = a.rP + ownerSlab + t;
                T part = zeroOf<T>();
                for (int k0 = tailFrom + lane; k0 < rowLen + (kTailUnroll - 1) * kWave; k0 += kTailUnroll * kWave) {
                    T tv[kTailUnroll];
                    int tc[kTailUnroll];
#pragma unroll
                    for (int u = 0; u < kTailUnroll; ++u) {
                        const int k = k0 + u * kWave;
                        const bool in = k < rowLen;
                        tv[u] = in ? rowVals[(long long)k * a.valStride] : zeroOf<T>();
                        tc[u] = in ? rowIdxs[(long long)k * a.idxStride] - a.baseIndex : -1;
                    }
                    T tx[kTailUnroll];
#pragma unroll
                    for (int u = 0; u < kTailUnroll; ++u)
                        tx[u] = x[tc[u] >= 0 ? tc[u] : 0];
#pragma unroll
                    for (int u = 0; u < kTailUnroll; ++u)
                        part = pick(tc[u] >= 0, mulAdd(tv[u], tx[u], part), part);
                }
#pragma unroll
                for (int m = 1; m < kWave; m <<= 1)
                    part = add(part, laneXor(part, m));
                if (lane == owner)
                    sum[t] = add(sum[t], part);
            }
        }
    }

#pragma unroll
    for (int m = LPC; m < kWave; m <<= 1) {
#pragma unroll
        for (int t = 0; t < RPL; ++t)
            sum[t] = add(sum[t], laneXor(sum[t], m));
    }

    if (phase != 0 || !stripLive)
        return;

    const bool hasBeta = isNotZero(a.beta);
    if (!a.rIdx && a.wideIO && row0 + RPL <= a.rows) {
        Pack<T, RPL> out;
        if (hasBeta) {
            const Pack<T, RPL> yv = loadPack<false, T, RPL>(a.y + row0);
#pragma unroll
            for (int t = 0; t < RPL; ++t)
                out.v[t] = epilogue<true>(a.alpha, sum[t], a.beta, yv.v[t]);
        } else {
#pragma unroll
            for (int t = 0; t < RPL; ++t)
                out.v[t] = epilogue<false>(a.alpha, sum[t], a.beta, zeroOf<T>());
        }
        storePack<T, RPL>(a.z + row0, out);
    } else {
#pragma unroll
        for (int t = 0; t < RPL; ++t) {
            const long long r = row0 + t;
            if (r < a.rows) {
                const int outRow = a.rIdx ? a.rIdx[r] : (int)r;
                a.z[outRow] = hasBeta ? epilogue<true>(a.alpha, sum[t], a.beta, a.y[outRow])
                                      : epilogue<false>(a.alpha, sum[t], a.beta, zeroOf<T>());
            }
        }
    }
    };

    for (int once = 0; once < 1; ++once)
        processGroup(groupOf());
}
```

spgpu_amd/csrc/spgpu_internal.h:

```cpp
#pragma once
#include "spgpu/core.h"
#include "spgpu/tuning.h"

#include <pthread.h>

#ifdef __cplusplus
extern "C" {
#endif

#define SPGPU_HANDLE_MAGIC 0x53504750u

#define SPGPU_REDUCE_MAX_BLOCKS 1024
#define SPGPU_REDUCE_SCRATCH_BYTES (SPGPU_REDUCE_MAX_BLOCKS * 16)

#define SPGPU_DEEP_STREAMS 8
#define SPGPU_PLANS 8
#define SPGPU_PLAN_WORDS 4
#define SPGPU_PLAN_GRAVES 32
typedef struct SpgpuPrivateHandle {
    SpgpuHandleStruct pub;
    unsigned magic;
    void* reduceScratch;
    void* reduceHost;
    int* formFeedback;
    const void* formKey[8];
    int formRows[8];
    int formCalls[8];
    int formGeneration[8];
    unsigned formNext;
    pthread_mutex_t tablesLock;
    int spmvForm;
    void* deepScratch[SPGPU_DEEP_STREAMS];
    hipStream_t deepStream[SPGPU_DEEP_STREAMS];
    hipEvent_t deepIdle[SPGPU_DEEP_STREAMS];
    int deepUsed[SPGPU_DEEP_STREAMS];
    int deepPinned[SPGPU_DEEP_STREAMS];
    unsigned deepClock[SPGPU_DEEP_STREAMS];
    unsigned deepTick;
    int deepStreams;
    int deepFallbacks;
    int deepRecycled;
    int lastSpmvForm;
    struct SpgpuSpmvPlan* plans;
    int* planPinned;
    void* planGraveyard[SPGPU_PLAN_GRAVES];
    int planGraves;
    unsigned planClock;
    int planUses, planBuilds, planStales;
    int planFreezes;
    struct SpgpuAdopted* adopted;
    int adoptedCount;
    int adoptedUses;
    int planFrozenSlabs;
} SpgpuPrivateHandle;
#define SPGPU_FEEDBACK_ENTRIES 8
#define SPGPU_FEEDBACK_SAMPLES 4

static inline SpgpuPrivateHandle* spgpuPrivate(spgpuHandle_t h)
{
    return (SpgpuPrivateHandle*)(void*)h;
}

typedef struct SpgpuDeepEntry {
    int row0;
    int depth;
    int firstItem;
    int items;
} SpgpuDeepEntry;
typedef struct SpgpuDeepItem {
    int row0;
    unsigned base;
    int depth;
    int chunk;
} SpgpuDeepItem;
#define SPGPU_DEEP_ENTRIES 8192
#define SPGPU_DEEP_ITEMS 20480
enum { SPGPU_DEEP_HEAD_ENTRIES = 0, SPGPU_DEEP_HEAD_ITEMS = 1, SPGPU_DEEP_HEAD_TICKET = 2, SPGPU_DEEP_HEAD_CUT = 3, SPGPU_DEEP_HEAD_INTS = 64 };
typedef struct SpgpuDeepList {
    int* header;
    SpgpuDeepEntry* entries;
    SpgpuDeepItem* items;
    void* partials;
    void* itemSums;
    hipEvent_t idle;
} SpgpuDeepList;
spgpuStatus_t spgpuDeepScratch(spgpuHandle_t h, SpgpuDeepList* list);
void spgpuDeepListPin(spgpuHandle_t h);

typedef struct SpgpuPlanBlock {
    int lowest, highest;
    int middle;
    int probed;
    unsigned long long deepMask;
    int firstDeep;
    int packBase;
} SpgpuPlanBlock;
typedef struct SpgpuSpmvPlan {
    const void *rP, *rS, *rIdx, *hackOffsets;
    long long idxStride;
    int rows, hackSize, baseIndex, maxNnz, deepCap, subs;
    int state;
    int stales;
    int uses;
    unsigned clock;
    int blocks;
    int deep;
    void* device;
    long long packedBytes;
    void* packed;
    int* pinned;
    hipEvent_t built;
    int holds;
} SpgpuSpmvPlan;
enum { SPGPU_PLAN_EMPTY = 0, SPGPU_PLAN_BUILDING = 1, SPGPU_PLAN_READY = 2, SPGPU_PLAN_GIVEN_UP = 3 };
void spgpuTablesLock(spgpuHandle_t h);
void spgpuTablesUnlock(spgpuHandle_t h);
SpgpuSpmvPlan* spgpuPlanRecord(spgpuHandle_t h, const SpgpuSpmvPlan* key);
SpgpuSpmvPlan* spgpuPlanFind(spgpuHandle_t h, const SpgpuSpmvPlan* key);
int spgpuPlanLanded(SpgpuSpmvPlan* plan, int wait);
void spgpuPlanCountFrozenSlabs(spgpuHandle_t h);
void spgpuRecordsCreate(SpgpuPrivateHandle* h);
void spgpuRecordsDestroy(SpgpuPrivateHandle* h);
#define SPGPU_ADOPTED 4
typedef struct SpgpuAdopted {
    const void *cM, *rP, *rS, *hackOffsets;
    int rows, hackSize, baseIndex, type;
    long long valPitch, idxPitch;
    void* values;
    int* indices;
    int* hackOffsetsOrdered;
    int* lengths;
    int* order;
    long long bytes;
    int holds;
} SpgpuAdopted;
const SpgpuAdopted* spgpuAdoptedFind(spgpuHandle_t h, hipStream_t stream, const void* cM, const int* rP, const int* rS, const int* hackOffsets,
                                     int rows, int hackSize, int baseIndex, long long valPitch, long long idxPitch);
int spgpuAdoptedAdd(spgpuHandle_t h, const SpgpuAdopted* entry);
int spgpuAdoptedRemove(spgpuHandle_t h, const int* rP, SpgpuAdopted* out);

int spgpuPlanTableHeld(spgpuHandle_t h);

void spgpuPlanRetire(spgpuHandle_t h, SpgpuSpmvPlan* plan);

static inline int spgpuEventDone(hipEvent_t event)
{
    const hipError_t said = hipEventQuery(event);
    if (said != hipSuccess && hipPeekAtLastError() == said)
        (void)hipGetLastError();
    return said == hipSuccess;
}

static inline int spgpuStreamCapturing(hipStream_t stream)
{
    hipStreamCaptureStatus status = hipStreamCaptureStatusNone;
    if (hipStreamIsCapturing(stream, &status) != hipSuccess) {
        (void)hipGetLastError();
        return 1;
    }
    return status != hipStreamCaptureStatusNone;
}

void spgpuDebugCheck(spgpuHandle_t h, const char* what);

void spgpuNoteSpmvForm(spgpuHandle_t h, int form);

int* spgpuFormFeedback(spgpuHandle_t h, const void* key, int rows, int* calls, int* tag);
static inline int spgpuFeedbackSaid(int word, int tag)
{
    return (word & ~0xFF) == tag ? (word & 0xFF) : 0;
}

typedef struct SpgpuTuning {
    int xStrips;
    int autoSweep;
    int poisonScratch;
    int deepSplit;
    int deepCap;
    int deepKeep;
    int raggedShape;
    int raggedSplit;
    int plan;
    int freezeEscapesPct;
} SpgpuTuning;
const SpgpuTuning* spgpuTuning(void);

int* spgpuAnalyseWords(spgpuHandle_t h);
int* spgpuDeepOverflowWords(spgpuHandle_t h);

#ifdef __cplusplus
}
#endif
```

Baseline: 1002 GFLOP/s.

## Process two slab groups per wave, prefetching the next group's first stage

Adds a multi-group slab kernel for fp64 in which each wave handles two consecutive row groups. The next group's first value/index stage is fetched during the last stage of the current group, so there is no load bubble at the group boundary and half as many blocks are launched. It is enabled automatically when the row count exceeds two groups per resident wave, or forced through an environment knob. The cost is more register pressure and possibly lower occupancy, which could reduce latency hiding in a bandwidth-bound kernel.

```diff
diff --git a/include/spgpu/ext/slab_groups.h b/include/spgpu/ext/slab_groups.h
--- /dev/null
+++ b/include/spgpu/ext/slab_groups.h
@@ -0,0 +1,13 @@
+#pragma once
+#include "../core.h"
+
+#ifdef __cplusplus
+extern "C" {
+#endif
+
+int spgpuSlabGroupsPerWave(int rows, int groupRows);
+int spgpuGetLastSlabGroups(spgpuHandle_t handle);
+
+#ifdef __cplusplus
+}
+#endif
diff --git a/spgpu_amd/capi.py b/spgpu_amd/capi.py
--- a/spgpu_amd/capi.py
+++ b/spgpu_amd/capi.py
@@ -274,6 +274,9 @@
 spgpuHellSpmvForm = _decl("spgpuHellSpmvForm", i32, [Handle, i32, ptr, i32, ptr, ptr, i32, i32])
 spgpuEllSpmvForm = _decl("spgpuEllSpmvForm", i32, [Handle, i32, ptr, i32, ptr, i32, i32, i32])
 
+spgpuSlabGroupsPerWave = _decl("spgpuSlabGroupsPerWave", i32, [i32, i32])
+spgpuGetLastSlabGroups = _decl("spgpuGetLastSlabGroups", i32, [Handle])
+
 spgpuTuningReload = _decl("spgpuTuningReload", None, [])
 
 
diff --git a/spgpu_amd/csrc/core.c b/spgpu_amd/csrc/core.c
--- a/spgpu_amd/csrc/core.c
+++ b/spgpu_amd/csrc/core.c
@@ -284,6 +284,16 @@
     __atomic_store_n(&spgpuPrivate(pHandle)->lastSpmvForm, form, __ATOMIC_RELAXED);
 }
 
+int spgpuGetLastSlabGroups(spgpuHandle_t pHandle)
+{
+    return __atomic_load_n(&spgpuPrivate(pHandle)->lastSlabGroups, __ATOMIC_RELAXED);
+}
+
+void spgpuNoteSlabGroups(spgpuHandle_t pHandle, int groups)
+{
+    __atomic_store_n(&spgpuPrivate(pHandle)->lastSlabGroups, groups, __ATOMIC_RELAXED);
+}
+
 static SpgpuTuning tuning;
 static int tuningLoaded;
 
@@ -297,6 +307,7 @@
 {
     SpgpuTuning t;
     t.xStrips = envInt("SPGPU_X_STRIPS", -1);
+    t.slabGroups = envInt("SPGPU_SLAB_GROUPS", 0);
     t.autoSweep = envInt("SPGPU_AUTO_SWEEP", 1);
     t.poisonScratch = envInt("SPGPU_POISON_SCRATCH", 0);
     t.deepSplit = envInt("SPGPU_DEEP_SPLIT", -1);
diff --git a/spgpu_amd/csrc/ellpack_spmv.hip b/spgpu_amd/csrc/ellpack_spmv.hip
--- a/spgpu_amd/csrc/ellpack_spmv.hip
+++ b/spgpu_amd/csrc/ellpack_spmv.hip
@@ -5,6 +5,7 @@
 
 #include "spgpu/ell.h"
 #include "spgpu/hell.h"
+#include "spgpu/ext/slab_groups.h"
 
 #include <stdio.h>
 #include <stdlib.h>
@@ -37,6 +38,16 @@
     const unsigned blocks = (unsigned)((groups + WAVES - 1) / WAVES);
     hipLaunchKernelGGL((slabSpmvKernel<T, RPL, PH, IS_HELL, NT, UNROLL, PIPE, TAIL, STRIPS, BLOCK, TILE_BYTES, TAIL_EVERY, PACKED>),
                        dim3(blocks), dim3(BLOCK), 0, stream, a);
+}
+
+template <typename T, int RPL, int PH, bool IS_HELL, int UNROLL, bool STRIPS, int GROUPS>
+static void launchSlabGroupsKernel(hipStream_t stream, const SlabArgs<T>& a)
+{
+    constexpr int GROUP_ROWS = (kWave / PH) * RPL;
+    constexpr int WAVES = kBlockThreads / kWave;
+    const long long groups = ((long long)a.rows + GROUP_ROWS - 1) / GROUP_ROWS;
+    const unsigned blocks = (unsigned)((groups + WAVES * GROUPS - 1) / (WAVES * GROUPS));
+    hipLaunchKernelGGL((slabGroupsSpmvKernel<T, RPL, PH, IS_HELL, true, UNROLL, true, STRIPS, GROUPS>), dim3(blocks), dim3(kBlockThreads), 0, stream, a);
 }
 
 template <typename T, int RPL, bool IS_HELL>
@@ -246,6 +257,16 @@
             } else {
                 findFrozenSlab(handle, stream, a, kWideGroupRows<T>);
                 constexpr int PH = PHASED ? 2 * WIDE : 1, UNROLL = PHASED ? 2 : 8;
+                if constexpr (std::is_same<T, double>::value) {
+                    if (!a.planPacked && spgpuSlabGroupsPerWave(a.rows, kWideGroupRows<T>) > 1) {
+                        spgpuNoteSlabGroups(handle, SPGPU_SLAB_GROUPS);
+                        if (vote.strips)
+                            launchSlabGroupsKernel<T, WIDE, PH, IS_HELL, UNROLL, true, SPGPU_SLAB_GROUPS>(stream, a);
+                        else
+                            launchSlabGroupsKernel<T, WIDE, PH, IS_HELL, UNROLL, false, SPGPU_SLAB_GROUPS>(stream, a);
+                        return;
+                    }
+                }
                 if (a.planPacked && vote.strips)
                     launchSlabKernel<T, WIDE, PH, IS_HELL, true, UNROLL, true, true, true, kBlockThreads, 0, 0, true>(stream, a);
                 else if (a.planPacked)
@@ -274,6 +295,8 @@
     hipStream_t stream = handle->currentStream;
     constexpr int WIDE = 16 / (int)sizeof(T);
     const bool wideOk = wideLayout<T, IS_HELL>(a);
+    if (call == SpmvCall::Run)
+        spgpuNoteSlabGroups(handle, 1);
     a.tailLanes = kTailLanes;
     int form = spgpuGetSpmvForm(handle);
     if (spgpuTuning()->xStrips >= 0)
@@ -462,6 +485,15 @@
 
 extern "C" {
 
+int spgpuSlabGroupsPerWave(int rows, int groupRows)
+{
+    const int asked = spgpuTuning()->slabGroups;
+    if (asked >= 1)
+        return asked == 1 ? 1 : SPGPU_SLAB_GROUPS;
+    const long long groups = groupRows > 0 ? ((long long)rows + groupRows - 1) / groupRows : 0;
+    return groups >= (long long)SPGPU_SLAB_GROUPS * SPGPU_RESIDENT_WAVES ? SPGPU_SLAB_GROUPS : 1;
+}
+
 int spgpuTuningVariantsBuilt(void)
 {
     return 0;
diff --git a/spgpu_amd/csrc/slab_spmv.hip.h b/spgpu_amd/csrc/slab_spmv.hip.h
--- a/spgpu_amd/csrc/slab_spmv.hip.h
+++ b/spgpu_amd/csrc/slab_spmv.hip.h
@@ -15,420 +15,14 @@
           int BLOCK = kBlockThreads, int TILE_BYTES = 0, int TAIL_EVERY = 0, bool PACKED = false>
 __global__ __launch_bounds__(BLOCK) void slabSpmvKernel(const SlabArgs<T> a)
 {
-    static_assert(!PACKED || (TILE_BYTES == 0 && RPL >= 2), "packed indices: the gather and strip forms of 4- and 8-byte elements");
-    using ColumnWord = typename std::conditional<PACKED, unsigned short, int>::type;
-    constexpr int LPC = kWave / PH;
-    constexpr int GROUP_ROWS = LPC * RPL;
-    constexpr int WAVES = BLOCK / kWave;
-    constexpr bool XTILE = TILE_BYTES > 0;
-    constexpr int TILE_ELEMS = TILE_BYTES / (int)sizeof(T);
+    constexpr int GROUPS = 1;
+#include "slab_spmv_body.hip.h"
+}
 
-    const int lane = threadIdx.x & (kWave - 1);
-    const int sub = lane % LPC;
-    const int phase = lane / LPC;
-    const T* __restrict__ x = a.x;
-    auto groupOf = [&]() -> long long {
-        const int wave = threadIdx.x >> 6;
-        return (long long)blockIdx.x * WAVES + wave;
-    };
-
-    T* tile = nullptr;
-    int tileBase = 0;
-    unsigned tileCount = 0;
-    if constexpr (XTILE) {
-        tile = ldsArray<T, TILE_ELEMS>();
-        ColumnProbe mine{0x7fffffff, -0x7fffffff - 1, 0, 0};
-        if (phase == 0) {
-            int first[RPL], last[RPL], lenAt[RPL];
-#pragma unroll
-            for (int once = 0; once < 1; ++once) {
-                const long long r0 = groupOf() * GROUP_ROWS + (long long)sub * RPL;
-                long long at = 0;
-                if (r0 < a.rows) {
-                    if constexpr (IS_HELL) {
-                        const unsigned u0 = (unsigned)r0, hs = (unsigned)a.hackSize;
-                        at = (long long)a.hackOffsets[u0 / hs] + (u0 % hs);
-                    } else {
-                        at = r0;
-                    }
-                }
-#pragma unroll
-                for (int t = 0; t < RPL; ++t) {
-                    const long long r = r0 + t;
-                    lenAt[t] = r < a.rows ? (a.rS ? a.rS[r] : a.maxNnz) : 0;
-                    first[t] = lenAt[t] > 0 ? a.rP[at + t] : 0;
-                    last[t] = lenAt[t] > 0 ? a.rP[at + t + (long long)(lenAt[t] - 1) * a.idxStride] : 0;
-                }
-            }
-#pragma unroll
-            for (int t = 0; t < RPL; ++t) {
-                if (lenAt[t] > 0) {
-                    const int f = first[t] - a.baseIndex, l = last[t] - a.baseIndex;
-                    const int low = f < l ? f : l, high = f < l ? l : f;
-                    mine.lowest = low < mine.lowest ? low : mine.lowest;
-                    mine.highest = high > mine.highest ? high : mine.highest;
-                    mine.middles += ((long long)f + l) >> 1;
-                    mine.rows += 1;
-                }
-            }
-        }
-        mine.lowest = waveMin(mine.lowest);
-        mine.highest = waveMax(mine.highest);
-#pragma unroll
-        for (int m = 1; m < kWave; m <<= 1) {
-            mine.rows += laneXor(mine.rows, m);
-            const int lowHalf = laneXor((int)(unsigned)(mine.middles & 0xffffffffll), m);
-            const int highHalf = laneXor((int)(mine.middles >> 32), m);
-            mine.middles += ((long long)highHalf << 32) | (unsigned)lowHalf;
-        }
-        ColumnProbe* seen = ldsArray<ColumnProbe, WAVES>();
-        if (lane == 0)
-            seen[threadIdx.x >> 6] = mine;
-        __syncthreads();
-        ColumnProbe all{0x7fffffff, -0x7fffffff - 1, 0, 0};
-#pragma unroll
-        for (int w = 0; w < WAVES; ++w) {
-            const ColumnProbe other = seen[w];
-            all.lowest = other.lowest < all.lowest ? other.lowest : all.lowest;
-            all.highest = other.highest > all.highest ? other.highest : all.highest;
-            all.rows += other.rows;
-            all.middles += other.middles;
-        }
-        if (all.rows > 0 && all.lowest >= 0) {
-            const long long span = (long long)all.highest - all.lowest + 1;
-            if (span <= TILE_ELEMS) {
-                tileBase = all.lowest;
-                tileCount = (unsigned)span;
-            } else {
-                long long start = all.middles / all.rows - TILE_ELEMS / 2;
-                start = start < all.lowest ? all.lowest : start;
-                start = start + TILE_ELEMS > (long long)all.highest + 1 ? (long long)all.highest + 1 - TILE_ELEMS : start;
-                tileBase = (int)start;
-                tileCount = TILE_ELEMS;
-            }
-        }
-        constexpr int PIECE = 16 / (int)sizeof(T);
-        const T* __restrict__ from = x + tileBase;
-        const unsigned pieces = tileCount / PIECE;
-        for (unsigned p0 = threadIdx.x; p0 < pieces; p0 += 4u * BLOCK) {
-            Pack<T, PIECE> w[4];
-#pragma unroll
-            for (int q = 0; q < 4; ++q)
-                if (p0 + q * BLOCK < pieces)
-                    w[q] = loadPackElementAligned<T, PIECE>(from + (size_t)(p0 + q * BLOCK) * PIECE);
-#pragma unroll
-            for (int q = 0; q < 4; ++q)
-                if (p0 + q * BLOCK < pieces)
-                    storePack<T, PIECE>(tile + (size_t)(p0 + q * BLOCK) * PIECE, w[q]);
-        }
-        if (pieces * PIECE + threadIdx.x < tileCount)
-            tile[pieces * PIECE + threadIdx.x] = from[pieces * PIECE + threadIdx.x];
-        __syncthreads();
-    }
-
-    auto processGroup = [&](const long long group) {
-    const long long groupRow0 = group * GROUP_ROWS;
-    if (groupRow0 >= a.rows)
-        return;
-    const long long row0 = groupRow0 + (long long)sub * RPL;
-    const bool stripLive = row0 < a.rows;
-
-    long long slab = 0;
-    if (stripLive) {
-        if constexpr (IS_HELL) {
-            const unsigned r0 = (unsigned)row0, hs = (unsigned)a.hackSize;
-            const unsigned hack = r0 / hs;
-            slab = (long long)a.hackOffsets[hack] + (r0 - hack * hs);
-        } else {
-            slab = row0;
-        }
-    }
-
-    int len[RPL];
-    int laneLongest = 0;
-#pragma unroll
-    for (int t = 0; t < RPL; ++t) {
-        const long long r = row0 + t;
-        len[t] = r < a.rows ? (a.rS ? a.rS[r] : a.maxNnz) : 0;
-        laneLongest = len[t] > laneLongest ? len[t] : laneLongest;
-    }
-    const int groupLongest = waveMax(laneLongest);
-
-    T sum[RPL];
-#pragma unroll
-    for (int t = 0; t < RPL; ++t)
-        sum[t] = zeroOf<T>();
-
-    const T* __restrict__ vals = a.cM + slab;
-    const int* __restrict__ idxs = a.rP + slab;
-    int packBase = 0;
-    if constexpr (PACKED)
-        packBase = a.packBases[group];
-
-    struct Stage {
-        Pack<T, RPL> v[UNROLL];
-        Pack<ColumnWord, RPL> c[UNROLL];
-    };
-    auto fetch = [&](int kBase, Stage& s) {
-#pragma unroll
-        for (int u = 0; u < UNROLL; ++u) {
-            const int k = kBase + u * PH + phase;
-            if (k < laneLongest) {
-                s.v[u] = loadPack<NT, T, RPL>(vals + (long long)k * a.valStride);
-                if constexpr (PACKED)
-                    s.c[u] = loadPack<NT, unsigned short, RPL>(a.planPacked + slab + (long long)k * a.idxStride);
-                else
-                    s.c[u] = loadPack<NT, int, RPL>(idxs + (long long)k * a.idxStride);
-            } else {
-#pragma unroll
-                for (int t = 0; t < RPL; ++t) {
-                    s.v[u].v[t] = zeroOf<T>();
-                    s.c[u].v[t] = PACKED ? (ColumnWord)0xFFFF : (ColumnWord)a.baseIndex;
-                }
-            }
-        }
-    };
-    auto columnOf = [&](const Stage& s, int u, int t, int k) -> int {
-        if constexpr (PACKED) {
-            const unsigned word = s.c[u].v[t];
-            if (word == 0xFFFFu)
-                return k < len[t] ? idxs[t + (long long)k * a.idxStride] - a.baseIndex : 0;
-            return packBase + (int)word;
-        } else {
-            return s.c[u].v[t] - a.baseIndex;
-        }
-    };
-    auto consume = [&](auto stripsTag, int kBase, const Stage& s, auto&& between) {
-        constexpr bool AS_STRIPS = decltype(stripsTag)::value;
-        T xv[UNROLL][RPL];
-        bool use[UNROLL][RPL];
-#pragma unroll
-        for (int u = 0; u < UNROLL; ++u) {
-            const int k = kBase + u * PH + phase;
-            if constexpr (AS_STRIPS) {
-                const bool present = k < len[0];
-                const Pack<T, RPL> w = loadPackElementAligned<T, RPL>(present ? x + (PACKED ? packBase + (int)s.c[u].v[0] : (int)s.c[u].v[0] - a.baseIndex) : a.cM);
-#pragma unroll
-                for (int t = 0; t < RPL; ++t) {
-                    use[u][t] = present;
-                    xv[u][t] = w.v[t];
-                }
-            } else if constexpr (XTILE) {
-                bool outside = false;
-                unsigned at[RPL];
-#pragma unroll
-                for (int t = 0; t < RPL; ++t) {
-                    const int col = s.c[u].v[t] - a.baseIndex;
-                    use[u][t] = k < len[t] && col >= 0;
-                    at[t] = (unsigned)(col - tileBase);
-                    const bool inside = at[t] < tileCount;
-                    outside |= use[u][t] && !inside;
-                    xv[u][t] = tile[inside ? at[t] : 0u];
-                }
-                if (__ballot(outside) != 0ull) {
-#pragma unroll
-                    for (int t = 0; t < RPL; ++t) {
-                        if (use[u][t] && at[t] >= tileCount)
-                            xv[u][t] = x[s.c[u].v[t] - a.baseIndex];
-                    }
-                }
-            } else {
-#pragma unroll
-                for (int t = 0; t < RPL; ++t) {
-                    const int col = columnOf(s, u, t, k);
-                    use[u][t] = k < len[t] && col >= 0;
-                    xv[u][t] = x[use[u][t] ? col : 0];
-                }
-            }
-        }
-        between();
-#pragma unroll
-        for (int u = 0; u < UNROLL; ++u) {
-#pragma unroll
-            for (int t = 0; t < RPL; ++t) {
-                sum[t] = pick(use[u][t], mulAdd(s.v[u].v[t], xv[u][t], sum[t]), sum[t]);
-            }
-        }
-    };
-    auto stageIsStrips = [&](int kBase, const Stage& s) -> bool {
-        bool scattered = false;
-#pragma unroll
-        for (int u = 0; u < UNROLL; ++u) {
-            const int k = kBase + u * PH + phase;
-            const bool present = k < len[0];
-#pragma unroll
-            for (int t = 0; t < RPL; ++t) {
-                if constexpr (PACKED)
-                    scattered |= (k < len[t]) != present ||
-                                 (present && (s.c[u].v[t] == 0xFFFFu || (unsigned)s.c[u].v[t] != (unsigned)s.c[u].v[0] + (unsigned)t));
-                else
-                    scattered |= (k < len[t]) != present ||
-                                 (present && (s.c[u].v[0] - a.baseIndex < 0 || s.c[u].v[t] != s.c[u].v[0] + t));
-            }
-        }
-        return __ballot(scattered) == 0ull;
-    };
-
-    auto columnSpan = [&]() -> long long {
-        int lowest = 0x7fffffff, highest = -1;
-        bool below = false;
-        if (phase == 0) {
-#pragma unroll
-            for (int t = 0; t < RPL; ++t) {
-                if (len[t] > 0) {
-                    const int f = idxs[t] - a.baseIndex, l = idxs[t + (long long)(len[t] - 1) * a.idxStride] - a.baseIndex;
-                    below |= f < 0 || l < 0;
-                    lowest = f < lowest ? f : lowest;
-                    lowest = l < lowest ? l : lowest;
-                    highest = f > highest ? f : highest;
-                    highest = l > highest ? l : highest;
-                }
-            }
-        }
-        lowest = waveMin(lowest);
-        highest = waveMax(highest);
-        if (__ballot(below) != 0ull)
-            return 1ll << 40;
-        return highest < lowest ? 0ll : (long long)highest - lowest + 1;
-    };
-
-    constexpr int STEP = PH * UNROLL;
-    int tailFrom = groupLongest;
-    constexpr int TAIL_STRIDE = TAIL_EVERY > 0 ? TAIL_EVERY : PH * UNROLL;
-    auto switchToTail = [&](int kBase) -> bool {
-        if constexpr (TAIL) {
-            if (kBase % TAIL_STRIDE == 0 && __popcll(__ballot(kBase < laneLongest)) <= a.tailLanes) {
-                tailFrom = kBase;
-                return true;
-            }
-        }
-        return false;
-    };
-    constexpr bool STRIPS_POSSIBLE = STRIPS && RPL > 1;
-    int kBase = 0;
-    bool done = false;
-    if constexpr (PIPE) {
-        Stage cur, nxt;
-        fetch(0, cur);
-        auto stage = [&](auto form) {
-            consume(form, kBase, cur, [&] { fetch(kBase + STEP, nxt); });
-            cur = nxt;
-        };
-        if constexpr (STRIPS_POSSIBLE) {
-            for (; kBase < groupLongest; kBase += STEP) {
-                if (switchToTail(kBase)) {
-                    done = true;
-                    break;
-                }
-                if (!stageIsStrips(kBase, cur))
-                    break;
-                stage(std::true_type{});
-            }
-            if (a.feedback) {
-                const long long groups = ((long long)a.rows + GROUP_ROWS - 1) / GROUP_ROWS;
-                if (group == sampleGroup(groups, 1) || group == sampleGroup(groups, 2) || group == sampleGroup(groups, 3)) {
-                    const int other = groupLongest > STEP && columnSpan() <= a.tileSpanLimit ? 3 : 1;
-                    for (int q = 1; q <= 3; ++q)
-                        if (group == sampleGroup(groups, q) && lane == 0)
-                            a.feedback[q - 1] = a.feedbackTag | (2 * kBase >= groupLongest && groupLongest > STEP ? 2 : other);
-                }
-            }
-        }
-        if (!done) {
-            for (kBase = __builtin_amdgcn_readfirstlane(kBase); kBase < groupLongest; kBase += STEP) {
-                if (switchToTail(kBase))
-                    break;
-                stage(std::false_type{});
-            }
-        }
-    } else {
-        for (; kBase < groupLongest; kBase += STEP) {
-            if (switchToTail(kBase))
-                break;
-            Stage cur;
-            fetch(kBase, cur);
-            consume(std::false_type{}, kBase, cur, [] {});
-        }
-    }
-
-    if constexpr (TAIL) {
-        unsigned long long pending = __ballot(tailFrom < laneLongest);
-        while (pending) {
-            const int owner = (__ffsll((long long)pending) - 1) % LPC;
-            pending &= ~__ballot(sub == owner);
-            const long long ownerSlab = __shfl(slab, owner, kWave);
-#pragma unroll
-            for (int t = 0; t < RPL; ++t) {
-                const int rowLen = __shfl(len[t], owner, kWave);
-                if (rowLen <= tailFrom)
-                    continue;
-                const T* __restrict__ rowVals = a.cM + ownerSlab + t;
-                const int* __restrict__ rowIdxs = a.rP + ownerSlab + t;
-                T part = zeroOf<T>();
-                for (int k0 = tailFrom + lane; k0 < rowLen + (kTailUnroll - 1) * kWave; k0 += kTailUnroll * kWave) {
-                    T tv[kTailUnroll];
-                    int tc[kTailUnroll];
-#pragma unroll
-                    for (int u = 0; u < kTailUnroll; ++u) {
-                        const int k = k0 + u * kWave;
-                        const bool in = k < rowLen;
-                        tv[u] = in ? rowVals[(long long)k * a.valStride] : zeroOf<T>();
-                        tc[u] = in ? rowIdxs[(long long)k * a.idxStride] - a.baseIndex : -1;
-                    }
-                    T tx[kTailUnroll];
-#pragma unroll
-                    for (int u = 0; u < kTailUnroll; ++u)
-                        tx[u] = x[tc[u] >= 0 ? tc[u] : 0];
-#pragma unroll
-                    for (int u = 0; u < kTailUnroll; ++u)
-                        part = pick(tc[u] >= 0, mulAdd(tv[u], tx[u], part), part);
-                }
-#pragma unroll
-                for (int m = 1; m < kWave; m <<= 1)
-                    part = add(part, laneXor(part, m));
-                if (lane == owner)
-                    sum[t] = add(sum[t], part);
-            }
-        }
-    }
-
-#pragma unroll
-    for (int m = LPC; m < kWave; m <<= 1) {
-#pragma unroll
-        for (int t = 0; t < RPL; ++t)
-            sum[t] = add(sum[t], laneXor(sum[t], m));
-    }
-
-    if (phase != 0 || !stripLive)
-        return;
-
-    const bool hasBeta = isNotZero(a.beta);
-    if (!a.rIdx && a.wideIO && row0 + RPL <= a.rows) {
-        Pack<T, RPL> out;
-        if (hasBeta) {
-            const Pack<T, RPL> yv = loadPack<false, T, RPL>(a.y + row0);
-#pragma unroll
-            for (int t = 0; t < RPL; ++t)
-                out.v[t] = epilogue<true>(a.alpha, sum[t], a.beta, yv.v[t]);
-        } else {
-#pragma unroll
-            for (int t = 0; t < RPL; ++t)
-                out.v[t] = epilogue<false>(a.alpha, sum[t], a.beta, zeroOf<T>());
-        }
-        storePack<T, RPL>(a.z + row0, out);
-    } else {
-#pragma unroll
-        for (int t = 0; t < RPL; ++t) {
-            const long long r = row0 + t;
-            if (r < a.rows) {
-                const int outRow = a.rIdx ? a.rIdx[r] : (int)r;
-                a.z[outRow] = hasBeta ? epilogue<true>(a.alpha, sum[t], a.beta, a.y[outRow])
-                                      : epilogue<false>(a.alpha, sum[t], a.beta, zeroOf<T>());
-            }
-        }
-    }
-    };
-
-    for (int once = 0; once < 1; ++once)
-        processGroup(groupOf());
+template <typename T, int RPL, int PH, bool IS_HELL, bool NT, int UNROLL, bool TAIL, bool STRIPS, int GROUPS, int BLOCK = kBlockThreads>
+__global__ __launch_bounds__(BLOCK) void slabGroupsSpmvKernel(const SlabArgs<T> a)
+{
+    constexpr bool PIPE = true, PACKED = false;
+    constexpr int TILE_BYTES = 0, TAIL_EVERY = 0;
+#include "slab_spmv_body.hip.h"
 }
diff --git a/spgpu_amd/csrc/slab_spmv_body.hip.h b/spgpu_amd/csrc/slab_spmv_body.hip.h
--- /dev/null
+++ b/spgpu_amd/csrc/slab_spmv_body.hip.h
@@ -0,0 +1,507 @@
+    static_assert(!PACKED || (TILE_BYTES == 0 && RPL >= 2), "packed indices: the gather and strip forms of 4- and 8-byte elements");
+    static_assert(GROUPS == 1 || (PIPE && TILE_BYTES == 0 && !PACKED), "several groups per wavefront: the prefetching gather and strip forms on the caller's indices");
+    using ColumnWord = typename std::conditional<PACKED, unsigned short, int>::type;
+    constexpr int LPC = kWave / PH;
+    constexpr int GROUP_ROWS = LPC * RPL;
+    constexpr int WAVES = BLOCK / kWave;
+    constexpr bool XTILE = TILE_BYTES > 0;
+    constexpr int TILE_ELEMS = TILE_BYTES / (int)sizeof(T);
+
+    const int lane = threadIdx.x & (kWave - 1);
+    const int sub = lane % LPC;
+    const int phase = lane / LPC;
+    const T* __restrict__ x = a.x;
+    auto groupOf = [&]() -> long long {
+        const int wave = threadIdx.x >> 6;
+        return (long long)blockIdx.x * WAVES + wave;
+    };
+
+    T* tile = nullptr;
+    int tileBase = 0;
+    unsigned tileCount = 0;
+    if constexpr (XTILE) {
+        tile = ldsArray<T, TILE_ELEMS>();
+        ColumnProbe mine{0x7fffffff, -0x7fffffff - 1, 0, 0};
+        if (phase == 0) {
+            int first[RPL], last[RPL], lenAt[RPL];
+#pragma unroll
+            for (int once = 0; once < 1; ++once) {
+                const long long r0 = groupOf() * GROUP_ROWS + (long long)sub * RPL;
+                long long at = 0;
+                if (r0 < a.rows) {
+                    if constexpr (IS_HELL) {
+                        const unsigned u0 = (unsigned)r0, hs = (unsigned)a.hackSize;
+                        at = (long long)a.hackOffsets[u0 / hs] + (u0 % hs);
+                    } else {
+                        at = r0;
+                    }
+                }
+#pragma unroll
+                for (int t = 0; t < RPL; ++t) {
+                    const long long r = r0 + t;
+                    lenAt[t] = r < a.rows ? (a.rS ? a.rS[r] : a.maxNnz) : 0;
+                    first[t] = lenAt[t] > 0 ? a.rP[at + t] : 0;
+                    last[t] = lenAt[t] > 0 ? a.rP[at + t + (long long)(lenAt[t] - 1) * a.idxStride] : 0;
+                }
+            }
+#pragma unroll
+            for (int t = 0; t < RPL; ++t) {
+                if (lenAt[t] > 0) {
+                    const int f = first[t] - a.baseIndex, l = last[t] - a.baseIndex;
+                    const int low = f < l ? f : l, high = f < l ? l : f;
+                    mine.lowest = low < mine.lowest ? low : mine.lowest;
+                    mine.highest = high > mine.highest ? high : mine.highest;
+                    mine.middles += ((long long)f + l) >> 1;
+                    mine.rows += 1;
+                }
+            }
+        }
+        mine.lowest = waveMin(mine.lowest);
+        mine.highest = waveMax(mine.highest);
+#pragma unroll
+        for (int m = 1; m < kWave; m <<= 1) {
+            mine.rows += laneXor(mine.rows, m);
+            const int lowHalf = laneXor((int)(unsigned)(mine.middles & 0xffffffffll), m);
+            const int highHalf = laneXor((int)(mine.middles >> 32), m);
+            mine.middles += ((long long)highHalf << 32) | (unsigned)lowHalf;
+        }
+        ColumnProbe* seen = ldsArray<ColumnProbe, WAVES>();
+        if (lane == 0)
+            seen[threadIdx.x >> 6] = mine;
+        __syncthreads();
+        ColumnProbe all{0x7fffffff, -0x7fffffff - 1, 0, 0};
+#pragma unroll
+        for (int w = 0; w < WAVES; ++w) {
+            const ColumnProbe other = seen[w];
+            all.lowest = other.lowest < all.lowest ? other.lowest : all.lowest;
+            all.highest = other.highest > all.highest ? other.highest : all.highest;
+            all.rows += other.rows;
+            all.middles += other.middles;
+        }
+        if (all.rows > 0 && all.lowest >= 0) {
+            const long long span = (long long)all.highest - all.lowest + 1;
+            if (span <= TILE_ELEMS) {
+                tileBase = all.lowest;
+                tileCount = (unsigned)span;
+            } else {
+                long long start = all.middles / all.rows - TILE_ELEMS / 2;
+                start = start < all.lowest ? all.lowest : start;
+                start = start + TILE_ELEMS > (long long)all.highest + 1 ? (long long)all.highest + 1 - TILE_ELEMS : start;
+                tileBase = (int)start;
+                tileCount = TILE_ELEMS;
+            }
+        }
+        constexpr int PIECE = 16 / (int)sizeof(T);
+        const T* __restrict__ from = x + tileBase;
+        const unsigned pieces = tileCount / PIECE;
+        for (unsigned p0 = threadIdx.x; p0 < pieces; p0 += 4u * BLOCK) {
+            Pack<T, PIECE> w[4];
+#pragma unroll
+            for (int q = 0; q < 4; ++q)
+                if (p0 + q * BLOCK < pieces)
+                    w[q] = loadPackElementAligned<T, PIECE>(from + (size_t)(p0 + q * BLOCK) * PIECE);
+#pragma unroll
+            for (int q = 0; q < 4; ++q)
+                if (p0 + q * BLOCK < pieces)
+                    storePack<T, PIECE>(tile + (size_t)(p0 + q * BLOCK) * PIECE, w[q]);
+        }
+        if (pieces * PIECE + threadIdx.x < tileCount)
+            tile[pieces * PIECE + threadIdx.x] = from[pieces * PIECE + threadIdx.x];
+        __syncthreads();
+    }
+
+    struct Stage {
+        Pack<T, RPL> v[UNROLL];
+        Pack<ColumnWord, RPL> c[UNROLL];
+    };
+    struct Head {
+        long long slab;
+        int len[RPL];
+    };
+    auto headOf = [&](const long long row0) -> Head {
+        Head h;
+        h.slab = 0;
+        if (row0 < a.rows) {
+            if constexpr (IS_HELL) {
+                const unsigned r0 = (unsigned)row0, hs = (unsigned)a.hackSize;
+                const unsigned hack = r0 / hs;
+                h.slab = (long long)a.hackOffsets[hack] + (r0 - hack * hs);
+            } else {
+                h.slab = row0;
+            }
+        }
+#pragma unroll
+        for (int t = 0; t < RPL; ++t) {
+            const long long r = row0 + t;
+            h.len[t] = r < a.rows ? (a.rS ? a.rS[r] : a.maxNnz) : 0;
+        }
+        return h;
+    };
+    auto longestOf = [&](const Head& h) -> int {
+        int longest = 0;
+#pragma unroll
+        for (int t = 0; t < RPL; ++t)
+            longest = h.len[t] > longest ? h.len[t] : longest;
+        return longest;
+    };
+    auto fetchFrom = [&](const long long from, const int longest, int kBase, Stage& s) {
+#pragma unroll
+        for (int u = 0; u < UNROLL; ++u) {
+            const int k = kBase + u * PH + phase;
+            if (k < longest) {
+                s.v[u] = loadPack<NT, T, RPL>(a.cM + from + (long long)k * a.valStride);
+                s.c[u] = loadPack<NT, ColumnWord, RPL>((const ColumnWord*)a.rP + from + (long long)k * a.idxStride);
+            } else {
+#pragma unroll
+                for (int t = 0; t < RPL; ++t) {
+                    s.v[u].v[t] = zeroOf<T>();
+                    s.c[u].v[t] = (ColumnWord)a.baseIndex;
+                }
+            }
+        }
+    };
+    struct Ahead {
+        Head head;
+        Stage first;
+    };
+    struct NoneAhead {};
+
+    auto processGroup = [&](const long long group, auto& ahead, const bool more) {
+    const long long groupRow0 = group * GROUP_ROWS;
+    if (groupRow0 >= a.rows)
+        return;
+    const long long row0 = groupRow0 + (long long)sub * RPL;
+    const bool stripLive = row0 < a.rows;
+
+    long long slab = 0;
+    if constexpr (GROUPS > 1) {
+        slab = ahead.head.slab;
+    } else if (stripLive) {
+        if constexpr (IS_HELL) {
+            const unsigned r0 = (unsigned)row0, hs = (unsigned)a.hackSize;
+            const unsigned hack = r0 / hs;
+            slab = (long long)a.hackOffsets[hack] + (r0 - hack * hs);
+        } else {
+            slab = row0;
+        }
+    }
+
+    int len[RPL];
+    int laneLongest = 0;
+#pragma unroll
+    for (int t = 0; t < RPL; ++t) {
+        const long long r = row0 + t;
+        if constexpr (GROUPS > 1)
+            len[t] = ahead.head.len[t];
+        else
+            len[t] = r < a.rows ? (a.rS ? a.rS[r] : a.maxNnz) : 0;
+        laneLongest = len[t] > laneLongest ? len[t] : laneLongest;
+    }
+    const int groupLongest = waveMax(laneLongest);
+    int aheadLongest = 0;
+    bool aheadFetched = false;
+    if constexpr (GROUPS > 1) {
+        ahead.head = headOf(more ? row0 + GROUP_ROWS : (long long)a.rows);
+        aheadLongest = longestOf(ahead.head);
+    }
+
+    T sum[RPL];
+#pragma unroll
+    for (int t = 0; t < RPL; ++t)
+        sum[t] = zeroOf<T>();
+
+    const T* __restrict__ vals = a.cM + slab;
+    const int* __restrict__ idxs = a.rP + slab;
+    int packBase = 0;
+    if constexpr (PACKED)
+        packBase = a.packBases[group];
+
+    auto fetch = [&](int kBase, Stage& s) {
+#pragma unroll
+        for (int u = 0; u < UNROLL; ++u) {
+            const int k = kBase + u * PH + phase;
+            if (k < laneLongest) {
+                s.v[u] = loadPack<NT, T, RPL>(vals + (long long)k * a.valStride);
+                if constexpr (PACKED)
+                    s.c[u] = loadPack<NT, unsigned short, RPL>(a.planPacked + slab + (long long)k * a.idxStride);
+                else
+                    s.c[u] = loadPack<NT, int, RPL>(idxs + (long long)k * a.idxStride);
+            } else {
+#pragma unroll
+                for (int t = 0; t < RPL; ++t) {
+                    s.v[u].v[t] = zeroOf<T>();
+                    s.c[u].v[t] = PACKED ? (ColumnWord)0xFFFF : (ColumnWord)a.baseIndex;
+                }
+            }
+        }
+    };
+    auto columnOf = [&](const Stage& s, int u, int t, int k) -> int {
+        if constexpr (PACKED) {
+            const unsigned word = s.c[u].v[t];
+            if (word == 0xFFFFu)
+                return k < len[t] ? idxs[t + (long long)k * a.idxStride] - a.baseIndex : 0;
+            return packBase + (int)word;
+        } else {
+            return s.c[u].v[t] - a.baseIndex;
+        }
+    };
+    auto consume = [&](auto stripsTag, int kBase, const Stage& s, auto&& between) {
+        constexpr bool AS_STRIPS = decltype(stripsTag)::value;
+        T xv[UNROLL][RPL];
+        bool use[UNROLL][RPL];
+#pragma unroll
+        for (int u = 0; u < UNROLL; ++u) {
+            const int k = kBase + u * PH + phase;
+            if constexpr (AS_STRIPS) {
+                const bool present = k < len[0];
+                const Pack<T, RPL> w = loadPackElementAligned<T, RPL>(present ? x + (PACKED ? packBase + (int)s.c[u].v[0] : (int)s.c[u].v[0] - a.baseIndex) : a.cM);
+#pragma unroll
+                for (int t = 0; t < RPL; ++t) {
+                    use[u][t] = present;
+                    xv[u][t] = w.v[t];
+                }
+            } else if constexpr (XTILE) {
+                bool outside = false;
+                unsigned at[RPL];
+#pragma unroll
+                for (int t = 0; t < RPL; ++t) {
+                    const int col = s.c[u].v[t] - a.baseIndex;
+                    use[u][t] = k < len[t] && col >= 0;
+                    at[t] = (unsigned)(col - tileBase);
+                    const bool inside = at[t] < tileCount;
+                    outside |= use[u][t] && !inside;
+                    xv[u][t] = tile[inside ? at[t] : 0u];
+                }
+                if (__ballot(outside) != 0ull) {
+#pragma unroll
+                    for (int t = 0; t < RPL; ++t) {
+                        if (use[u][t] && at[t] >= tileCount)
+                            xv[u][t] = x[s.c[u].v[t] - a.baseIndex];
+                    }
+                }
+            } else {
+#pragma unroll
+                for (int t = 0; t < RPL; ++t) {
+                    const int col = columnOf(s, u, t, k);
+                    use[u][t] = k < len[t] && col >= 0;
+                    xv[u][t] = x[use[u][t] ? col : 0];
+                }
+            }
+        }
+        between();
+#pragma unroll
+        for (int u = 0; u < UNROLL; ++u) {
+#pragma unroll
+            for (int t = 0; t < RPL; ++t) {
+                sum[t] = pick(use[u][t], mulAdd(s.v[u].v[t], xv[u][t], sum[t]), sum[t]);
+            }
+        }
+    };
+    auto stageIsStrips = [&](int kBase, const Stage& s) -> bool {
+        bool scattered = false;
+#pragma unroll
+        for (int u = 0; u < UNROLL; ++u) {
+            const int k = kBase + u * PH + phase;
+            const bool present = k < len[0];
+#pragma unroll
+            for (int t = 0; t < RPL; ++t) {
+                if constexpr (PACKED)
+                    scattered |= (k < len[t]) != present ||
+                                 (present && (s.c[u].v[t] == 0xFFFFu || (unsigned)s.c[u].v[t] != (unsigned)s.c[u].v[0] + (unsigned)t));
+                else
+                    scattered |= (k < len[t]) != present ||
+                                 (present && (s.c[u].v[0] - a.baseIndex < 0 || s.c[u].v[t] != s.c[u].v[0] + t));
+            }
+        }
+        return __ballot(scattered) == 0ull;
+    };
+
+    auto columnSpan = [&]() -> long long {
+        int lowest = 0x7fffffff, highest = -1;
+        bool below = false;
+        if (phase == 0) {
+#pragma unroll
+            for (int t = 0; t < RPL; ++t) {
+                if (len[t] > 0) {
+                    const int f = idxs[t] - a.baseIndex, l = idxs[t + (long long)(len[t] - 1) * a.idxStride] - a.baseIndex;
+                    below |= f < 0 || l < 0;
+                    lowest = f < lowest ? f : lowest;
+                    lowest = l < lowest ? l : lowest;
+                    highest = f > highest ? f : highest;
+                    highest = l > highest ? l : highest;
+                }
+            }
+        }
+        lowest = waveMin(lowest);
+        highest = waveMax(highest);
+        if (__ballot(below) != 0ull)
+            return 1ll << 40;
+        return highest < lowest ? 0ll : (long long)highest - lowest + 1;
+    };
+
+    constexpr int STEP = PH * UNROLL;
+    int tailFrom = groupLongest;
+    constexpr int TAIL_STRIDE = TAIL_EVERY > 0 ? TAIL_EVERY : PH * UNROLL;
+    auto switchToTail = [&](int kBase) -> bool {
+        if constexpr (TAIL) {
+            if (kBase % TAIL_STRIDE == 0 && __popcll(__ballot(kBase < laneLongest)) <= a.tailLanes) {
+                tailFrom = kBase;
+                return true;
+            }
+        }
+        return false;
+    };
+    constexpr bool STRIPS_POSSIBLE = STRIPS && RPL > 1;
+    int kBase = 0;
+    bool done = false;
+    if constexpr (PIPE) {
+        Stage cur, nxt;
+        if constexpr (GROUPS > 1)
+            cur = ahead.first;
+        else
+            fetch(0, cur);
+        auto stage = [&](auto form) {
+            if constexpr (GROUPS > 1) {
+                const bool last = kBase + STEP >= groupLongest;
+                consume(form, kBase, cur, [&] {
+                    fetchFrom(last ? ahead.head.slab : slab, last ? aheadLongest : laneLongest, last ? 0 : kBase + STEP, nxt);
+                });
+                aheadFetched = last;
+            } else {
+                consume(form, kBase, cur, [&] { fetch(kBase + STEP, nxt); });
+            }
+            cur = nxt;
+        };
+        if constexpr (STRIPS_POSSIBLE) {
+            for (; kBase < groupLongest; kBase += STEP) {
+                if (switchToTail(kBase)) {
+                    done = true;
+                    break;
+                }
+                if (!stageIsStrips(kBase, cur))
+                    break;
+                stage(std::true_type{});
+            }
+            if (a.feedback) {
+                const long long groups = ((long long)a.rows + GROUP_ROWS - 1) / GROUP_ROWS;
+                if (group == sampleGroup(groups, 1) || group == sampleGroup(groups, 2) || group == sampleGroup(groups, 3)) {
+                    const int other = groupLongest > STEP && columnSpan() <= a.tileSpanLimit ? 3 : 1;
+                    for (int q = 1; q <= 3; ++q)
+                        if (group == sampleGroup(groups, q) && lane == 0)
+                            a.feedback[q - 1] = a.feedbackTag | (2 * kBase >= groupLongest && groupLongest > STEP ? 2 : other);
+                }
+            }
+        }
+        if (!done) {
+            for (kBase = __builtin_amdgcn_readfirstlane(kBase); kBase < groupLongest; kBase += STEP) {
+                if (switchToTail(kBase))
+                    break;
+                stage(std::false_type{});
+            }
+        }
+        if constexpr (GROUPS > 1) {
+            if (!aheadFetched)
+                fetchFrom(ahead.head.slab, aheadLongest, 0, cur);
+            ahead.first = cur;
+        }
+    } else {
+        for (; kBase < groupLongest; kBase += STEP) {
+            if (switchToTail(kBase))
+                break;
+            Stage cur;
+            fetch(kBase, cur);
+            consume(std::false_type{}, kBase, cur, [] {});
+        }
+    }
+
+    if constexpr (TAIL) {
+        unsigned long long pending = __ballot(tailFrom < laneLongest);
+        while (pending) {
+            const int owner = (__ffsll((long long)pending) - 1) % LPC;
+            pending &= ~__ballot(sub == owner);
+            const long long ownerSlab = __shfl(slab, owner, kWave);
+#pragma unroll
+            for (int t = 0; t < RPL; ++t) {
+                const int rowLen = __shfl(len[t], owner, kWave);
+                if (rowLen <= tailFrom)
+                    continue;
+                const T* __restrict__ rowVals = a.cM + ownerSlab + t;
+                const int* __restrict__ rowIdxs = a.rP + ownerSlab + t;
+                T part = zeroOf<T>();
+                for (int k0 = tailFrom + lane; k0 < rowLen + (kTailUnroll - 1) * kWave; k0 += kTailUnroll * kWave) {
+                    T tv[kTailUnroll];
+                    int tc[kTailUnroll];
+#pragma unroll
+                    for (int u = 0; u < kTailUnroll; ++u) {
+                        const int k = k0 + u * kWave;
+                        const bool in = k < rowLen;
+                        tv[u] = in ? rowVals[(long long)k * a.valStride] : zeroOf<T>();
+                        tc[u] = in ? rowIdxs[(long long)k * a.idxStride] - a.baseIndex : -1;
+                    }
+                    T tx[kTailUnroll];
+#pragma unroll
+                    for (int u = 0; u < kTailUnroll; ++u)
+                        tx[u] = x[tc[u] >= 0 ? tc[u] : 0];
+#pragma unroll
+                    for (int u = 0; u < kTailUnroll; ++u)
+                        part = pick(tc[u] >= 0, mulAdd(tv[u], tx[u], part), part);
+                }
+#pragma unroll
+                for (int m = 1; m < kWave; m <<= 1)
+                    part = add(part, laneXor(part, m));
+                if (lane == owner)
+                    sum[t] = add(sum[t], part);
+            }
+        }
+    }
+
+#pragma unroll
+    for (int m = LPC; m < kWave; m <<= 1) {
+#pragma unroll
+        for (int t = 0; t < RPL; ++t)
+            sum[t] = add(sum[t], laneXor(sum[t], m));
+    }
+
+    if (phase != 0 || !stripLive)
+        return;
+
+    const bool hasBeta = isNotZero(a.beta);
+    if (!a.rIdx && a.wideIO && row0 + RPL <= a.rows) {
+        Pack<T, RPL> out;
+        if (hasBeta) {
+            const Pack<T, RPL> yv = loadPack<false, T, RPL>(a.y + row0);
+#pragma unroll
+            for (int t = 0; t < RPL; ++t)
+                out.v[t] = epilogue<true>(a.alpha, sum[t], a.beta, yv.v[t]);
+        } else {
+#pragma unroll
+            for (int t = 0; t < RPL; ++t)
+                out.v[t] = epilogue<false>(a.alpha, sum[t], a.beta, zeroOf<T>());
+        }
+        storePack<T, RPL>(a.z + row0, out);
+    } else {
+#pragma unroll
+        for (int t = 0; t < RPL; ++t) {
+            const long long r = row0 + t;
+            if (r < a.rows) {
+                const int outRow = a.rIdx ? a.rIdx[r] : (int)r;
+                a.z[outRow] = hasBeta ? epilogue<true>(a.alpha, sum[t], a.beta, a.y[outRow])
+                                      : epilogue<false>(a.alpha, sum[t], a.beta, zeroOf<T>());
+            }
+        }
+    }
+    };
+
+    if constexpr (GROUPS > 1) {
+        const long long first = groupOf() * GROUPS;
+        Ahead ahead;
+        ahead.head = headOf(first * GROUP_ROWS + (long long)sub * RPL);
+        fetchFrom(ahead.head.slab, longestOf(ahead.head), 0, ahead.first);
+#pragma unroll 1
+        for (int g = 0; g < GROUPS; ++g)
+            processGroup(first + g, ahead, g + 1 < GROUPS);
+    } else {
+        NoneAhead none;
+        for (int once = 0; once < 1; ++once)
+            processGroup(groupOf(), none, false);
+    }
diff --git a/spgpu_amd/csrc/spgpu_internal.h b/spgpu_amd/csrc/spgpu_internal.h
--- a/spgpu_amd/csrc/spgpu_internal.h
+++ b/spgpu_amd/csrc/spgpu_internal.h
@@ -41,6 +41,7 @@
     int deepFallbacks;
     int deepRecycled;
     int lastSpmvForm;
+    int lastSlabGroups;
     struct SpgpuSpmvPlan* plans;
     int* planPinned;
     void* planGraveyard[SPGPU_PLAN_GRAVES];
@@ -164,6 +165,9 @@
 void spgpuDebugCheck(spgpuHandle_t h, const char* what);
 
 void spgpuNoteSpmvForm(spgpuHandle_t h, int form);
+void spgpuNoteSlabGroups(spgpuHandle_t h, int groups);
+#define SPGPU_SLAB_GROUPS 2
+#define SPGPU_RESIDENT_WAVES 3072
 
 int* spgpuFormFeedback(spgpuHandle_t h, const void* key, int rows, int* calls, int* tag);
 static inline int spgpuFeedbackSaid(int word, int tag)
@@ -173,6 +177,7 @@
 
 typedef struct SpgpuTuning {
     int xStrips;
+    int slabGroups;
     int autoSweep;
     int poisonScratch;
     int deepSplit;
```

After: 929.5 GFLOP/s. -7.2%, worse.
